# romz-pl/linear-programming-Vanderbei

Hardware: AMD Instinct MI355X
Metric: IPM iterations/sec (ADA^T factor+solve) on netlib dfl001; duality gap ≤1e-8 (higher is better)
Workload: dtype f64; 1 GPU; dfl001 hsd (BASELINE configs[2]), one step = one complete solve to mu < 1e-12; method=hsd, m=12155, n=12230, nz=71277, parallelism=replicas1, status=optimal solution, lnz=7160813, nsup=18147, levels=20, refine_passes=251

## Files before the change

### include/ipo_hip.h

```cpp
#ifndef IPO_HIP_H
#define IPO_HIP_H

#include <stdio.h>

#ifdef __cplusplus
extern "C" {
#endif

int solver(int m, int n, int nz, int *iA, int *kA, double *A, double *b, double *c, double f,
           double *x, double *y, double *w, double *z);

void ldltfac(int m, int n, int *kA, int *iA, double *A, double *dn, double *dm,
             int *kAt, int *iAt, double *At, int verbose);
void forwardbackward(double *Dn, double *Dm, double *dx, double *dy);
void inv_clo(void);
int ipo_hip_ldlt_set_q(int n, const int *kQ, const int *iQ, const double *Q, int max);

typedef struct {
    int    iters;
    int    status;
    double t_setup_s;
    double t_solve_s;
    double factor_ms;
    double solve_ms;
// ... 29 lines not shown
int  ipo_hip_ctx_run(ipo_hip_ctx *ctx, int method, int max_iter, FILE *trace, int timing, ipo_hip_stats *stats);
void ipo_hip_ctx_download(ipo_hip_ctx *ctx, double *x, double *y, double *w, double *z);
void ipo_hip_ctx_destroy(ipo_hip_ctx *ctx);
double ipo_hip_ctx_setup_seconds(const ipo_hip_ctx *ctx);

int ipo_hip_solve_qp(int m, int n, int nz, const int *iA, const int *kA, const double *A, const double *b,
                     const double *c, double f, const int *kQ, const int *iQ, const double *Q, double *x,
                     double *y, double *w, double *z, FILE *trace, int max_iter, int timing,
                     ipo_hip_stats *stats);
ipo_hip_ctx *ipo_hip_ctx_create_qp(int m, int n, const int *kA, const int *iA, const double *A,
                                   const double *b, const double *c, double f, const int *kQ, const int *iQ,
                                   const double *Q);

typedef int (*ipo_hip_allreduce_fn)(void *user, double *buf, long n, int op);
int ipo_hip_set_device(int device);
int ipo_hip_rccl_unique_id(void *out128);
ipo_hip_ctx *ipo_hip_ctx_create_shard(int m, int n, const int *kA, const int *iA, const double *A,
                                      const double *b, const double *c, double f, int nlink,
                                      int m_global, int n_global, long nz_global, int nranks, int rank,
                                      const void *rccl_id, ipo_hip_allreduce_fn fn, void *user);

int ipo_hip_run_mps(const char *path, int method, FILE *out, int timing, ipo_hip_stats *stats);

#define IPO_HIP_SPLIT_FREE 1
int ipo_hip_run_mps_ex(const char *path, int method, int flags, const char *solfile, FILE *out, int timing,
                       ipo_hip_stats *stats);

int ipo_hip_mps_dims(const char *path, int *m0, int *n0, int *nz0, int *m, int *n, int *nz);

int ipo_hip_mps_load(const char *path, int *m, int *n, int *nz, int *kA, int *iA, double *A,
                     double *b, double *c, double *f);

int ipo_hip_write_sol(const char *path, int flags, const double *x, const double *y, const double *z,
                      const char *solfile);

int ipo_hip_mps_quads(const char *path, int *n, int *qnz, int *kQ, int *iQ, double *Q);

int ipo_hip_mps_load_qp(const char *path, int *m, int *n, int *nz, int *kA, int *iA, double *A, double *b,
                        double *c, double *f, int *qnz, int *kQ, int *iQ, double *Q);

int ipo_hip_mps_load_ex(const char *path, int flags, int *m, int *n, int *nz, int *kA, int *iA, double *A,
                        double *b, double *c, double *f);

typedef struct ipo_hip_kkt ipo_hip_kkt;
ipo_hip_kkt *ipo_hip_kkt_create(int m, int n, const int *kA, const int *iA, const double *A);
ipo_hip_kkt *ipo_hip_kkt_create_q(int m, int n, const int *kA, const int *iA, const double *A, const int *kQ,
                                  const int *iQ, const double *Q, int qmax);
void   ipo_hip_kkt_destroy(ipo_hip_kkt *k);
int    ipo_hip_kkt_factor(ipo_hip_kkt *k, const double *E, const double *D);
int    ipo_hip_kkt_solve(ipo_hip_kkt *k, const double *E, const double *D, double *fy, double *fx);
int    ipo_hip_kkt_info(const ipo_hip_kkt *k, long *lnz, double *narth, int *nsup, int *nlevels, int *denwin,
                        int *pdf, double *epsdiag, int *ndep, int *passes);
int    ipo_hip_kkt_perm(const ipo_hip_kkt *k, int *perm);
int    ipo_hip_kkt_pivots(const ipo_hip_kkt *k, double *d, int *live);
void   ipo_hip_kkt_set_epsdiag(ipo_hip_kkt *k, double epsdiag);

int ipo_hip_symbolic(int m, int n, const int *kA, const int *iA, int *perm, long *lnz, double *narth,
                     int *denwin, int *pdf, int *nsup, int *nlevels);
int ipo_hip_symbolic_q(int m, int n, const int *kA, const int *iA, const int *kQ, const int *iQ, int *perm,
                       long *lnz, double *narth, int *denwin, int *pdf, int *nsup, int *nlevels);
int ipo_hip_symbolic_forced(int m, int n, const int *kA, const int *iA, int nforced, int *perm, int *colcount,
                            long *lnz, int *tail_c0, int *nsup, int *nlevels);
int ipo_hip_symbolic_tail(int m, int n, const int *kA, const int *iA, double density, int *tail_c0, int *nt,
                          int *ntb);

int ipo_hip_vector_bench(int m, int n, const int *kA, const int *iA, const double *A, int reps, double *ms3,
                         double *bytes3);

int ipo_hip_dot_ordered(const double *a, const double *b, int n, double *out);

int ipo_hip_q_times(int n, const int *kQ, const int *iQ, const double *Q, const double *v, int long_min,
                    double *out);
int ipo_hip_kkt_q_long(const ipo_hip_kkt *k);
int ipo_hip_ctx_q_long(const ipo_hip_ctx *ctx);

int ipo_hip_synth_random(int m, int n, int per_col, int band, unsigned long long seed, int *nz, int *kA, int *iA,
                         double *A, double *b, double *c, double *xs, double *ys, double *ws, double *zs);
int ipo_hip_synth_block_angular(int nblocks, int mb, int nb, int per_col, int band, int nlink, int link_nz,
                                unsigned long long seed, int *m, int *n, int *nz, int *kA, int *iA, double *A,
                                double *b, double *c, double *xs, double *ys, double *ws, double *zs);

int ipo_hip_tail_run_schedule(int nt, int K, int L, int cap, unsigned *items, int max_items, int *ptr);

long ipo_hip_kkt_schedule(int m, int n, const int *kA, const int *iA, int nforced, int cus, const char *name, int *out,
                          long cap);

int ipo_hip_device_count(void);
int ipo_hip_device_synchronize(void);
const char *ipo_hip_last_error(void);
const char *ipo_hip_version(void);

#ifdef __cplusplus
}
#endif
#endif
```

### linear-programming-vanderbei_amd/csrc/capi.cpp

```cpp
#include "../../include/ipo_hip.h"

#include <hip/hip_runtime.h>

#include <algorithm>
#include <cmath>
#include <cstdlib>
#include <cstring>
#include <memory>
#include <stdexcept>
#include <string>
#include <utility>
#include <vector>

#include "ipm.h"
#include "kkt_device.h"
#include "kkt_schedule.h"
#include "lp_io.h"
#include "synth.h"

namespace {

thread_local std::string g_err;

void set_err(const std::string& s) { g_err = s; }
// ... 733 lines not shown

int ipo_hip_device_synchronize(void) {
    const hipError_t e = hipDeviceSynchronize();
    if (e != hipSuccess) {
        set_err(std::string("hipDeviceSynchronize: ") + hipGetErrorString(e));
        return -1;
    }
    return 0;
}

const char* ipo_hip_last_error(void) { return g_err.c_str(); }
const char* ipo_hip_version(void) { return "ipo-hip 0.1 (gfx950)"; }

}

namespace {
std::vector<int> schedule_array(const ipo::KktPlan& P, const ipo::KktKnobs& knobs, const ipo::KktSchedule& S,
                                const std::string& name) {
    using V = std::vector<int>;
    const auto flat2 = [](const std::vector<ipo::SchedInt2>& w) {
        V v;
        for (const ipo::SchedInt2& e : w) { v.push_back(e.x); v.push_back(e.y); }
        return v;
    };
    const auto chars = [](const std::vector<char>& w) { return V(w.begin(), w.end()); };
    const auto one = [](size_t x) { return static_cast<int>(x); };
    const std::pair<const char*, const V*> direct[] = {
        {"plan.col0", &P.col0}, {"plan.rowptr", &P.rowptr}, {"plan.parent", &P.parent}, {"plan.level", &P.level},
        {"plan.level_ptr", &P.level_ptr}, {"plan.level_sups", &P.level_sups}, {"plan.sup_of", &P.sup_of},
        {"plan.yrow_ptr", &P.yrow_ptr}, {"plan.yrow_idx", &P.yrow_idx}, {"plan.unit_level_ptr", &P.unit_level_ptr},
        {"plan.unit_sup", &P.unit_sup}, {"plan.kslot", &P.kslot}, {"plan.kslot_ptr", &P.kslot_ptr},
        {"plan.tail_kslot_ptr", &P.tail_kslot_ptr},
        {"panels.fu_sup", &S.panels.fu_sup}, {"panels.fu_j", &S.panels.fu_j}, {"panels.small_sups", &S.panels.small_sups},
        {"panels.fu_ptr", &S.panels.fu_ptr}, {"panels.small_ptr", &S.panels.small_ptr},
        {"panels.small1_cnt", &S.panels.small1_cnt},
        {"chunks.chunk_sup", &S.chunks.chunk_sup}, {"chunks.chunk_r0", &S.chunks.chunk_r0},
        {"chunks.sup_chunk0", &S.chunks.sup_chunk0}, {"chunks.chunk_ptr", &S.chunks.chunk_ptr},
        {"order.sweep_sups", &S.order.sweep_sups}, {"order.leaf_cnt", &S.order.leaf_cnt},
        {"order.leaf8_cnt", &S.order.leaf8_cnt},
        {"sf.ybase", &S.sf.ybase}, {"sf.yrow_idx", &S.sf.yrow_idx}, {"sf.zbase", &S.sf.zbase}, {"sf.zpi", &S.sf.zpi},
        {"sf.need", &S.sf.need}, {"sf.par", &S.sf.par}, {"sf.ylate_ptr", &S.sf.ylate_ptr},
        {"sf.ylate_idx", &S.sf.ylate_idx}, {"sf.pre_col", &S.sf.pre_col}, {"sf.pre_ptr", &S.sf.pre_ptr},
        {"sf.pre_idx", &S.sf.pre_idx},
        {"visits.kslot", &S.visits.kslot}, {"visits.kptr", &S.visits.kptr}, {"visits.late_b", &S.visits.late_b},
        {"gather.ck_u", &S.gather.ck_u}, {"gather.ck_b", &S.gather.ck_b}, {"gather.ck_e", &S.gather.ck_e},
        {"gather.ck_part", &S.gather.ck_part}, {"gather.ck_q", &S.gather.ck_q}, {"gather.sp_u", &S.gather.sp_u},
        {"gather.sp_p0", &S.gather.sp_p0}, {"gather.sp_n", &S.gather.sp_n}, {"gather.ck_ptr", &S.gather.ck_ptr},
        {"gather.sp_ptr", &S.gather.sp_ptr}, {"gather.ck_kind", &S.gather.ck_kind},
        {"tail.visit_ptr", &S.tail.visit_ptr}, {"tail.run_ptr", &S.tail.run_ptr},
    };
    for (const auto& d : direct)
        if (name == d.first) return *d.second;
    if (name == "plan.dims") return {P.T, P.nsup, P.nlevels, P.tail_c0, P.nt, P.ntb};
    if (name == "plan.task_src") {
        V v;
        for (const ipo::TailTask& t : P.utasks) v.push_back(t.src);
        return v;
    }
    if (name == "paths")
        return {S.paths.visits, S.paths.chain_lead, S.paths.tail_run, S.paths.run_winpub, S.paths.small_leaves,
                S.paths.sf_width};
    if (name == "panels.split_level") return chars(S.panels.split_level);
    if (name == "sf.items_f") return flat2(S.sf.items_f);
    if (name == "sf.items_b") return flat2(S.sf.items_b);
    if (name == "sf.dims") return {S.sf.sf_level, one(S.sf.ybuf_stride), one(S.sf.zpad_stride), S.sf.late_lists};
    if (name == "visits.vis") {
        V v;
        for (size_t g = 0; g < S.visits.vis.size(); g++)
            for (const ipo::SchedInt3& e : S.visits.vis[g]) v.insert(v.end(), {one(g), e.x, e.y, e.z});
        return v;
    }
    if (name == "gather.ck_wide") return chars(S.gather.ck_wide);
    if (name == "gather.dims") return {one(S.gather.split_cnt), one(S.gather.partial_tiles)};
    if (name == "chunks.dims") return {one(S.chunks.partial_stride)};
    if (name == "work.launches") return {S.work.fwd_launches, S.work.bwd_launches};
    const auto steps = [](const std::vector<ipo::SweepStep>& w) {
        V v;
        for (const ipo::SweepStep& e : w) v.insert(v.end(), {e.kind, e.q0, e.n, e.a, e.b});
        return v;
    };
    if (name == "sweep.fwd") return steps(S.sweep.fwd);
    if (name == "sweep.bwd") return steps(S.sweep.bwd);
    if (name == "sweep.split") return {S.sweep.split};
    if (name == "sweep.fwd_blocked" || name == "sweep.bwd_blocked") {
        const ipo::SweepSteps b = ipo::build_sweep_steps(P, knobs, S.paths, S.chunks, S.order, S.sf, true);
        return steps(name == "sweep.fwd_blocked" ? b.fwd : b.bwd);
    }
    if (name == "tail.visit_list") return V(S.tail.visit_list.begin(), S.tail.visit_list.end());
    if (name == "tail.run_items") {
        V v;
        for (const ipo::SchedUint2& e : S.tail.run_items) { v.push_back(static_cast<int>(e.x)); v.push_back(static_cast<int>(e.y)); }
        return v;
    }
    throw std::invalid_argument("kkt_schedule: unknown array '" + name + "'");
}

void synth_out(const ipo::SynthLP& o, int* kA, int* iA, double* A, double* b, double* c, double* xs, double* ys,
               double* ws, double* zs) {
    std::copy(o.kA.begin(), o.kA.end(), kA);
    std::copy(o.iA.begin(), o.iA.end(), iA);
    std::copy(o.A.begin(), o.A.end(), A);
    std::copy(o.b.begin(), o.b.end(), b);
    std::copy(o.c.begin(), o.c.end(), c);
    if (xs) std::copy(o.xs.begin(), o.xs.end(), xs);
    if (ys) std::copy(o.ys.begin(), o.ys.end(), ys);
    if (ws) std::copy(o.ws.begin(), o.ws.end(), ws);
    if (zs) std::copy(o.zs.begin(), o.zs.end(), zs);
}
}

extern "C" {

int ipo_hip_vector_bench(int m, int n, const int* kA, const int* iA, const double* A, int reps, double* ms3,
                         double* bytes3) {
    try {
        ipo::vector_bench(m, n, kA, iA, A, reps, ms3, bytes3);
        return 0;
    } catch (const std::exception& e) {
        set_err(e.what());
        return -1;
    }
}

int ipo_hip_tail_run_schedule(int nt, int K, int L, int cap, unsigned* items, int max_items, int* ptr) {
    try {
        if (nt <= 0 || K <= 0 || L <= 0 || cap <= 1) throw std::invalid_argument("tail_schedule: bad arguments");
        const int ntb = (nt + ipo::kPanelCols - 1) / ipo::kPanelCols;
        if (ntb > ipo::kTailSchedMaxBlocks)
            throw std::invalid_argument("tail_schedule: nt gives " + std::to_string(ntb) + " block columns, the limit is " +
                                        std::to_string(ipo::kTailSchedMaxBlocks));
        std::vector<int> pv;
        const std::vector<ipo::SchedUint2> v = ipo::tail_run_schedule(ntb, nt, K, L, cap, pv);
        const int n = static_cast<int>(v.size());
        if (items)
            for (int i = 0; i < std::min(n, max_items); i++) {
                items[2 * i] = v[i].x;
                items[2 * i + 1] = v[i].y;
            }
        if (ptr) std::copy(pv.begin(), pv.end(), ptr);
        return n;
    } catch (const std::exception& e) {
        set_err(e.what());
        return -1;
    }
}

long ipo_hip_kkt_schedule(int m, int n, const int* kA, const int* iA, int nforced, int cus, const char* name, int* out,
                          long cap) {
    try {
        if (!name || cus <= 0) throw std::invalid_argument("kkt_schedule: bad arguments");
        std::vector<int> kat, iat;
        std::vector<double> at, a(kA[n], 1.0);
        ipo::csc_transpose(m, n, kA, iA, a.data(), kat, iat, at);
        const ipo::KktPlan P =
            ipo::build_kkt_plan(m, n, kA, iA, kat.data(), iat.data(), nforced, ipo::device_tail_density());
        const ipo::KktKnobs knobs = ipo::KktKnobs::from_env();
        const ipo::KktSchedule S = ipo::build_kkt_schedule(P, knobs, cus);
        const std::string names(name);
        std::vector<int> v;
        if (names.find(',') == std::string::npos) {
            v = schedule_array(P, knobs, S, names);
        } else {
            for (size_t b = 0; b <= names.size();) {
                const size_t e = std::min(names.find(',', b), names.size());
                const std::vector<int> w = schedule_array(P, knobs, S, names.substr(b, e - b));
                v.push_back(static_cast<int>(w.size()));
                v.insert(v.end(), w.begin(), w.end());
                b = e + 1;
            }
        }
        if (out) std::copy(v.begin(), v.begin() + std::min<long>(cap, static_cast<long>(v.size())), out);
        return static_cast<long>(v.size());
    } catch (const std::exception& e) {
        set_err(e.what());
        return -1;
    }
}

int ipo_hip_dot_ordered(const double* a, const double* b, int n, double* out) {
    try {
        if (n < 0 || (n > 0 && (!a || !b)) || !out) throw std::invalid_argument("dot_ordered: bad arguments");
        *out = ipo::dot_ordered_host(a, b, n);
        return 0;
    } catch (const std::exception& e) {
        set_err(e.what());
        return -1;
    }
}

int ipo_hip_q_times(int n, const int* kQ, const int* iQ, const double* Q, const double* v, int long_min,
                    double* out) {
    try {
        if (n < 0 || !kQ || !out || (n > 0 && !v)) throw std::invalid_argument("q_times: bad arguments");
        if (kQ[0] != 0) throw std::invalid_argument("q_times: kQ[0] != 0");
        for (int j = 0; j < n; j++)
            if (kQ[j + 1] < kQ[j]) throw std::invalid_argument("q_times: kQ decreasing at column " + std::to_string(j));
        if (n > 0 && kQ[n] > 0 && (!iQ || !Q)) throw std::invalid_argument("q_times: bad arguments");
        for (int k = 0; k < (n > 0 ? kQ[n] : 0); k++)
            if (iQ[k] < 0 || iQ[k] >= n) throw std::invalid_argument("q_times: row index out of range at entry " + std::to_string(k));
        const int thr = long_min > 0 ? long_min : ipo::KktKnobs::from_env().q_long;
        ipo::q_times_host(n, kQ, iQ, Q, v, thr, out);
        return 0;
    } catch (const std::exception& e) {
        set_err(e.what());
        return -1;
    }
}

int ipo_hip_kkt_q_long(const ipo_hip_kkt* k) { return k->kkt->q_long_count(); }

int ipo_hip_ctx_q_long(const ipo_hip_ctx* ctx) { return ctx->solver->kkt().q_long_count(); }

int ipo_hip_synth_random(int m, int n, int per_col, int band, unsigned long long seed, int* nz, int* kA, int* iA,
                         double* A, double* b, double* c, double* xs, double* ys, double* ws, double* zs) {
    try {
        if (nz) *nz = static_cast<int>(static_cast<long long>(n) * per_col);
        if (!kA) return 0;
        ipo::SynthLP o;
        ipo::synth_random(m, n, per_col, band, seed, o);
        synth_out(o, kA, iA, A, b, c, xs, ys, ws, zs);
        return 0;
    } catch (const std::exception& e) {
        set_err(e.what());
// ... 25 lines not shown
```

### linear-programming-vanderbei_amd/csrc/kkt_dense.hip

```cpp
#include <hip/hip_runtime.h>

#include <algorithm>
#include <cmath>
#include <stdexcept>

#include "dev_common.h"
#include "hip_util.h"
#include "kkt_kernels.h"

namespace ipo {

namespace {

struct DiagCtx {
    double* dscale;
    double* dg;
    int* live;
    int* flags;
    const int* sign;
    double tau;
};

__device__ __forceinline__ bool factor_diag_fast(const DiagCtx p, double* panel, int ld, int nc, int c0,
                                                 double (*B)[PC + 1]) {
// ... 877 lines not shown
            __builtin_amdgcn_s_setprio(3);
            if (cw0 + WIN <= nc) win_solve<true, DEP>(a, cw0, nc, rok, lane, Ct, Lb, dv, S.prog + w, prog + w, ds);
            else win_solve<false, DEP>(a, cw0, nc, rok, lane, Ct, Lb, dv, S.prog + w, prog + w, ds);
            if (SC && rp.pub && kb + 1 < tv.ntb) {
                bool ok = true;
                if (!DEP) {
                    for (int v = 0; v <= w; v++) {
                        int x;
                        while ((x = __hip_atomic_load(S.wverd + v, __ATOMIC_RELAXED, __HIP_MEMORY_SCOPE_WORKGROUP)) == 0)
                            __builtin_amdgcn_s_sleep(1);
                        ok = ok && x == 1;
                    }
                }
                if (ok && kb - 1 > rp.t0) {
                    const int need = max(1, (tv.nt - (kb - 1) * PC + TR - 1) / TR - 1);
                    int got = 0;
                    if (lane == 0) {
                        for (;;) {
                            got = sc1_load_int(rp.pread + kb - 1);
                            if (got >= need) break;
                            const int b = sc1_load_int(p.flags + 2);
                            if (b && b - 1 < kb) break;
                            __builtin_amdgcn_s_sleep(1);
                        }
                    }
                    ok = __builtin_amdgcn_readfirstlane(got) >= need;
                }
                if (ok) {
                    double* pb = rp.pub + (((size_t)(kb & 1) * tv.ntb + j) * 4 + w) * kTailPubWin;
                    if (rok) {
#pragma unroll
                        for (int q = 0; q < WIN; q++)
                            if (cw0 + q < nc) sc1_store(pb + q * TR + lane, a[q]);
                    }
                    if (lane < WIN) sc1_store(pb + WIN * TR + lane, dv[cw0 + lane]);
                    asm volatile("s_waitcnt vmcnt(0)" ::: "memory");
                    if (lane == 0)
                        __hip_atomic_store(rp.wflag_w + ((size_t)kb * tv.ntb + j) * 4 + w, rp.epoch, __ATOMIC_RELAXED,
                                           __HIP_MEMORY_SCOPE_AGENT);
                }
            }
        }
        __builtin_amdgcn_s_setprio(0);
        PANEL_STAMP(2);
        if (wbuf && (h1 ? rok : (j == 0 && lane >= nc && lane < h0))) {
            double dw[WIN];
            win_row(&dv[cw0], dw);
#pragma unroll
            for (int q = 0; q < WIN; q++) {
                const int c = cw0 + q;
                if (c < nc) wbuf[row + (size_t)c * ld] = a[q] * dw[q];
            }
        }
    }
    __builtin_amdgcn_fence(__ATOMIC_RELEASE, "workgroup", "local");
    __builtin_amdgcn_s_barrier();
    __builtin_amdgcn_fence(__ATOMIC_ACQUIRE, "workgroup", "local");
    if (winpub && !pre_wait()) return false;
    PANEL_STAMP(12);
    if (!DEP && tiny_sh && dep) return true;
    const bool fail = DEP ? (S.spec > 0 || (S.spec < 0 && S.ndep > 0 && [&] {
                                 for (int k = 0; k < nc; k++)
                                     if (!S.lv[k]) return true;
                                 return false;
                             }()))
                          : tiny_sh != 0;
    if (fail) {
        if (tid == 0) {
            atomicOr(&p.flags[1], fu_sup ? 2 : DEP ? 4 | 16 : 4);
            if (!fu_sup) atomicMax(&p.flags[2], kb + 1);
            if (DEP && !fu_sup && j == 0)
                __hip_atomic_store(p.flags + 3, 0, __ATOMIC_RELAXED, __HIP_MEMORY_SCOPE_AGENT);
        }
        post(true);
        return false;
    }
    if (w < nwin && (h1 ? rok && tile : (j == 0 && lane >= nc && lane < h0))) {
#pragma unroll
        for (int q = 0; q < WIN; q++) {
            const int c = cw0 + q;
            if (c < nc) st_h<SC>(panel + row + (size_t)c * ld, a[q]);
        }
    }
    if (j == 0 && tid < nc) { st_h<SC>(p.dg + c0 + tid, dv[tid]); p.live[c0 + tid] = DEP ? S.lv[tid] != 0 : 1; }
    post(false);
    if (!fu_sup && pre && j == 0 && !h1 && lane < nc && (lane >> 4) == w) st_h<SC>(p.dscale + c0 + lane, dsc_pre);
    if (j != 0) return false;
    if (!h1) {
#pragma unroll
        for (int q = 0; q < WIN; q++) Ct[lane][cw0 + q] = a[q];
    }
    __syncthreads();
    for (int rr = 1 + wv; rr < nc; rr += PNT / 64)
        if (lane < rr) st_h<SC>(panel + lane + (size_t)rr * ld, Ct[rr][lane]);
    if (DEP && tid == 0) {
        if (S.ndep) atomicAdd(&p.flags[0], S.ndep);
        if (!fu_sup)
            __hip_atomic_store(p.flags + 3, S.ndep, __ATOMIC_RELAXED, __HIP_MEMORY_SCOPE_AGENT);
    }
    PANEL_STAMP(13);
    return false;
}

__global__ void __launch_bounds__(PNT)
k_panel_w(PlanView p, const int* __restrict__ fu_sup, const int* __restrict__ fu_j, int f0, TailView tv, int kb) {
    __shared__ __attribute__((aligned(16))) char lds[sizeof(PanelLds)];
    PanelLds& S = *reinterpret_cast<PanelLds*>(lds);
    const int dep = fu_sup ? (tv.sdep ? 1 : 0) : 0;
    if (panel_w_body<false>(p, fu_sup, fu_j, f0, tv, kb, blockIdx.x, S, tv.W, false, nullptr, 0, dep)) {
        __syncthreads();
        panel_w_body<true>(p, fu_sup, fu_j, f0, tv, kb, blockIdx.x, S, tv.W, false, nullptr, 0, dep);
    }
}


constexpr int SKS = PC + 16;
struct SyrkLds {
    double As[PC][SKS];
    double Bs[PC][SKS];
};

template <int S>
__device__ __forceinline__ double diag_terms(const double (*As)[S], const double (*Bs)[S], int r, int nc, double as) {
    int k = 0;
    for (; k + 16 <= nc; k += 16) {
        double pr[16];
#pragma unroll
        for (int u = 0; u < 16; u++) pr[u] = fabs(As[k + u][r] * Bs[k + u][r]);
#pragma unroll
        for (int u = 0; u < 16; u++) as += pr[u];
    }
    for (; k < nc; k++) as += fabs(As[k][r] * Bs[k][r]);
    return as;
}
__device__ __forceinline__ double diag_terms(const SyrkLds& L, int r, int nc, double as) {
    return diag_terms<SKS>(L.As, L.Bs, r, nc, as);
}

__device__ __forceinline__ void mfma_32x16(const SyrkLds& L, int wr, int wc, int li, int lk, double4_t (&acc)[2]) {
#pragma unroll
    for (int kk = 0; kk < PC; kk += 4) {
        double av[2];
#pragma unroll
        for (int a = 0; a < 2; a++) av[a] = L.As[kk + lk][wr + a * 16 + li];
        const double bv = L.Bs[kk + lk][wc + li];
#pragma unroll
        for (int a = 0; a < 2; a++) acc[a] = __builtin_amdgcn_mfma_f64_16x16x4f64(av[a], bv, acc[a], 0, 0, 0);
    }
}

#ifdef IPO_VISIT_STAMPS
__device__ long long g_vstamps[8][16][6];
#define VISIT_STAMP(blk, slot)                                                                          \
    do {                                                                                                \
        if (blockIdx.x == 0 && (threadIdx.x & 63) == 0 && (blk) < 16)                                   \
            g_vstamps[threadIdx.x >> 6][(blk)][(slot)] = clock64();                                     \
    } while (0)
#else
#define VISIT_STAMP(blk, slot) do {} while (0)
#endif

__device__ __forceinline__ void syrk_tile512(const PlanView& p, const TailView& tv, int kb, int bi, int bj,
                                             SyrkLds& L) {
    const int nt = tv.nt, k0 = kb * PC, nc = min(PC, nt - k0), tid = threadIdx.x;
    const double* Lcol = tv.S + (size_t)k0 * nt;
    {
        double va[TR * PC / PNT], vb[TR * PC / PNT];
// ... 119 lines not shown
        __syncthreads();
        VISIT_STAMP(b - b0, 2);
        if (b + 1 < b1) load(b + 1, xx, yy, dd);
        VISIT_STAMP(b - b0, 3);
        mfma_32x16(L, wr, wc, li, lk, acc);
        VISIT_STAMP(b - b0, 4);
        if (diag_tile && tid < TR) as = diag_terms(L, tid, min(PC, nt - b * PC), as);
        __syncthreads();
        VISIT_STAMP(b - b0, 5);
    };
    for (int b = b0; b < b1; b++) step(b, rx, ry, rd);
#pragma unroll
    for (int a = 0; a < 2; a++)
#pragma unroll
        for (int i = 0; i < 4; i++) L.As[wc + (lane & 15)][wr + a * 16 + (lane >> 4) + 4 * i] = acc[a][i];
    __syncthreads();
#pragma unroll
    for (int u = 0; u < 8; u++) {
        const int cc = wv + 8 * u, cg = bj * TR + cc;
        if (rgl < nt && cg < nt && !(diag_tile && cc > lane)) st_h<SC>(tv.S + rgl + (size_t)cg * nt, old[u] - L.As[cc][lane]);
    }
    if (diag_tile && tid < TR && bi * TR + tid < nt) {
        double* dp = p.dscale + tv.tc + bi * TR + tid;
        st_h<SC>(dp, ld_h<SC>(dp) + as);
    }
}

constexpr size_t kTailStepLds0 = sizeof(PanelLds) > sizeof(SyrkLds) ? sizeof(PanelLds) : sizeof(SyrkLds);
constexpr size_t kTailStepLds = kTailStepLds0 > sizeof(PreLds) ? kTailStepLds0 : sizeof(PreLds);

__global__ void __launch_bounds__(PNT)
k_tail_pr(PlanView p, TailView tv, int t, int gp, int vbase) {
    __shared__ __attribute__((aligned(16))) char lds[kTailStepLds];
    if ((int)blockIdx.x < gp) {
        PanelLds& S = *reinterpret_cast<PanelLds*>(lds);
        if (panel_w_body<false>(p, nullptr, nullptr, 0, tv, t, blockIdx.x, S, nullptr, t > 0, p.flags + 2, t, tv.dep)) {
            __syncthreads();
            panel_w_body<true>(p, nullptr, nullptr, 0, tv, t, blockIdx.x, S, nullptr, t > 0, p.flags + 2, t, tv.dep);
        }
        return;
    }
    if (tv.vlist) {
        const unsigned v = tv.vlist[vbase + blockIdx.x - gp];
        visit_tile512(p, tv, v & 255, (v >> 8) & 255, (v >> 16) & 255, v >> 24, *reinterpret_cast<SyrkLds*>(lds),
                      p.flags + 2, t);
        return;
    }
    int tile = blockIdx.x - gp, c = t + 1;
    while (tile >= tv.ntb - c) { tile -= tv.ntb - c; c++; }
    const int b1 = visit_hi(t, c, tv.vk);
    visit_tile512(p, tv, c + tile, c, max(0, b1 - tv.vk), b1, *reinterpret_cast<SyrkLds*>(lds), p.flags + 2, t);
}

__host__ __device__ __forceinline__ int tail_gp(int nt, int t) { return max(1, (nt - t * PC + TR - 1) / TR - 1); }

__global__ void __launch_bounds__(PNT)
k_tail_run(PlanView p, TailView tv, TailRun rc) {
    __shared__ __attribute__((aligned(16))) char lds[kTailStepLds];
    __shared__ int sh_item, sh_ok, sh_ok2;
    const int ntb = tv.ntb;
    const int* bailp = p.flags + 2;
    if (threadIdx.x == 0) sh_item = __hip_atomic_fetch_add(rc.ticket, 1, __ATOMIC_RELAXED, __HIP_MEMORY_SCOPE_AGENT);
    __syncthreads();
    const int it = sh_item;
    if (it >= rc.n) return;
    const uint2 rec = rc.items[it];
    const int t = rec.y & 0xff, q = (rec.y >> 8) & 0xff;
    unsigned long long* tr = rc.trace ? rc.trace + 4 * (size_t)it : nullptr;
    if (tr && threadIdx.x == 0) {
        tr[0] = __builtin_amdgcn_s_memrealtime();
        tr[3] = __builtin_amdgcn_s_getreg((20 << 0) | (0 << 6) | (3 << 11));
    }
    if (rec.y >> 31) {
        const int j = rec.x;
        const int* vd = q ? rc.vseq + t * ntb + t : nullptr;
        const int* vt = q && t + j + 1 < ntb ? rc.vseq + (t + j + 1) * ntb + t : nullptr;
        const bool winpub = rc.pub && t > 0 && t - 1 >= rc.t0;
        if (!winpub && !run_wait(vd, q, vt, q, bailp, t, &sh_ok)) return;
        auto pw = [&]() {
            const bool go = t == rc.t0 || run_wait(rc.pdone + t - 1, tail_gp(tv.nt, t - 1), nullptr, 0, bailp, t, &sh_ok2);
            if (tr && threadIdx.x == 0) tr[1] = __builtin_amdgcn_s_memrealtime();
            return go;
        };
        auto post = [&](bool bailed) { run_signal(rc.pdone + t, bailed ? 1 + kRunBail : 1); };
        if (tr && threadIdx.x == 0 && t == 0) tr[1] = __builtin_amdgcn_s_memrealtime();
        PanelLds& S = *reinterpret_cast<PanelLds*>(lds);
        const RunPub rp{rc.pub, rc.wflag, rc.wflag, rc.pread, rc.t0, rc.epoch, vd, vt, q, &sh_ok};
        if (panel_w_body<false, true>(p, nullptr, nullptr, 0, tv, t, j, S, nullptr, t > 0, nullptr, t, tv.dep, pw,
                                      post, rp)) {
            __syncthreads();
            panel_w_body<true, true>(p, nullptr, nullptr, 0, tv, t, j, S, nullptr, t > 0, nullptr, t, tv.dep, NoWait{},
                                     post, rp);
        }
    } else {
        const int bi = rec.x & 255, c = (rec.x >> 8) & 255, b0 = (rec.x >> 16) & 255, b1 = rec.x >> 24;
        int* vs = rc.vseq + bi * ntb + c;
        if (!run_wait(t > rc.t0 ? rc.pdone + t - 1 : nullptr, t > rc.t0 ? tail_gp(tv.nt, t - 1) : 0, q ? vs : nullptr,
                      q, bailp, t, &sh_ok))
            return;
        if (tr && threadIdx.x == 0) tr[1] = __builtin_amdgcn_s_memrealtime();
        visit_tile512<true>(p, tv, bi, c, b0, b1, *reinterpret_cast<SyrkLds*>(lds));
        run_signal(vs);
    }
    if (tr && threadIdx.x == 0) tr[2] = __builtin_amdgcn_s_memrealtime();
}

__global__ void __launch_bounds__(256)
k_tail_restore(PlanView p, TailView tv, int kb) {
    const int nt = tv.nt, k0 = kb * PC, nc = min(PC, nt - k0), h = nt - k0, c = blockIdx.y;
    double* panel = tv.S + k0 + (size_t)k0 * nt;
    for (int row = nc + blockIdx.x * 256 + threadIdx.x; row < h; row += gridDim.x * 256)
        panel[row + (size_t)c * nt] = tv.W[row + (size_t)c * nt];
    if (blockIdx.x == 0 && c == 0) {
        if ((int)threadIdx.x < nc) p.dscale[tv.tc + k0 + threadIdx.x] = tv.W[threadIdx.x];
        if (threadIdx.x == 0) {
            p.flags[0] -= p.flags[3];
            p.flags[3] = 0;
        }
    }
}

__global__ void __launch_bounds__(PNT)
k_tail_col(PlanView p, TailView tv, int t) {
    __shared__ __attribute__((aligned(16))) char lds[sizeof(SyrkLds)];
    syrk_tile512(p, tv, t, t + 1 + blockIdx.x, t + 1, *reinterpret_cast<SyrkLds*>(lds));
}

constexpr int SNC = 16;

__device__ __forceinline__ void panel_s_body(const PlanView& p, const int* __restrict__ sups, int q0, int q, int dep) {
    const int lane = threadIdx.x & 63;
    const int s = sups[q0 + q];
    const int c0 = p.col0[s], nc = p.col0[s + 1] - c0;
    const int h = nc + (p.rowptr[s + 1] - p.rowptr[s]), ld = h;
    double* panel = p.Lx + p.off[s];
    const bool rok = lane < h;
    double a[SNC];
#pragma unroll
    for (int c = 0; c < SNC; c++) {
        const bool ok = rok && c < nc && c <= lane;
        const double t = panel[ok ? lane + (size_t)c * ld : 0];
        a[c] = ok ? t : 0.0;
    }
    double dsc = lane < nc ? p.dscale[c0 + lane] : 0.0;
    double mydv = 0.0;
    int mylive = 1, ndep = 0;
#pragma unroll
    for (int k = 0; k < SNC; k++) {
        if (k < nc) {
            double dk = lane_bcast(a[k], k);
            const double dsk = lane_bcast(dsc, k);
            int alive = 1;
            if (fabs(dk) <= p.tau * dsk) {
                const bool in = lane > k && rok;
                const bool nan = __ballot(in && a[k] != a[k]) != 0;
                if (!dep || nan) {
                    if (lane == 0) atomicOr(&p.flags[1], 8);
                    return;
                }
                if (__ballot(in && !(fabs(a[k]) < 1.0e+6 * 1.0e-8)) != 0) dk = (p.sign[c0 + k] < 0 ? -1.0 : 1.0) * 1.0e-8;
                else alive = 0;
                ndep++;
            }
            mylive = lane == k ? alive : mylive;
            const bool below = lane > k && rok;
            const double l = alive && below ? a[k] / dk : 0.0;
            a[k] = below ? l : a[k];
            mydv = lane == k ? dk : mydv;
            const double c = l * dk;
            dsc = dsc + fabs(l * c);
#pragma unroll
            for (int qq = k + 1; qq < SNC; qq++)
                if (qq < nc) a[qq] = a[qq] - l * lane_bcast(c, qq);
        }
    }
    if (rok) {
// ... 154 lines not shown
```

### linear-programming-vanderbei_amd/csrc/kkt_device.h

```cpp
#pragma once
#include <hip/hip_runtime.h>

#include <cstddef>
#include <cstdint>
#include <memory>
#include <vector>

#include "hip_util.h"
#include "exchange.h"
#include "kkt_knobs.h"
#include "kkt_plan.h"
#include "kkt_schedule.h"

namespace ipo {

struct TailView {
    double* S;
    int nt, ntb, tc;
    const int* task_ptr;
    const TailTask* tasks;
    double* W;
    int vk = kTailVisitBlocks;
    int dep = 1;
    const unsigned* vlist = nullptr;
    const int* vptr = nullptr;
    int sdep = 1;
};

struct TailRun {
    const uint2* items;
    int n;
    int t0;
    int* ticket;
    int* pdone;
    int* vseq;
    double* pub = nullptr;
    int* wflag = nullptr;
    int* pread = nullptr;
    int epoch = 0;
    unsigned long long* trace = nullptr;
};

constexpr int kTailPubWin = 16 * 64 + 16;

struct KktTimers {
    double phase_ms[kNumPhases] = {};
    long phase_launches[kNumPhases] = {};
    long phase_count[kNumPhases] = {};
    double factor_ms = 0.0;
    double solve_ms = 0.0;
    double sweep_ms = 0.0;
    long factors = 0, solves = 0, rawsolves = 0;
    long panel_redos = 0;
    long redo_where[4] = {0, 0, 0, 0};
    long tail_repairs = 0;
    long tail_dep_rounds = 0;
};

struct QBlock {
    const int* kQ = nullptr;
    const int* iQ = nullptr;
    const double* Q = nullptr;
    int qmax = 1;
};

struct PlanView;

class KktDevice {
  public:
    KktDevice(int m, int n, const int* kA, const int* iA, const double* A, hipStream_t stream, int nforced = 0,
              const QBlock* qb = nullptr);
    ~KktDevice();
    KktDevice(const KktDevice&) = delete;
    KktDevice& operator=(const KktDevice&) = delete;

    const KktPlan& plan() const { return plan_; }
    void set_exchange(Exchange* x) { xch_ = x; }
    int nforced() const { return nforced_; }
    int m() const { return m_; }
    int n() const { return n_; }
    hipStream_t stream() const { return stream_; }

    const int* kA() const { return dkA_.get(); }
    const int* iA() const { return diA_.get(); }
    const double* A() const { return dA_.get(); }
    const int* kAt() const { return dkAt_.get(); }
    const int* iAt() const { return diAt_.get(); }
    const double* At() const { return dAt_.get(); }
    const int* kQ() const { return qnz_ > 0 ? dkQ_.get() : nullptr; }
    const int* iQ() const { return qnz_ > 0 ? diQ_.get() : nullptr; }
    const double* Q() const { return qnz_ > 0 ? dQ_.get() : nullptr; }
    int q_long_count() const { return q_long_n_; }
    int q_long_min() const { return q_long_n_ > 0 ? knobs_.q_long : 0; }
    void launch_q_long(const double* v, double* out);

    struct PrePass {
        int R = 0;
        double* dfy[2] = {nullptr, nullptr};
        double* dfx[2] = {nullptr, nullptr};
        hipStream_t stream = nullptr;
        hipEvent_t ready = nullptr;
    };
    void factor(const double* dE, const double* dD, const PrePass* pre = nullptr);
    int solve(const double* dE, const double* dD, double* dfy, double* dfx);
    int solve2(const double* dE, const double* dD, double* dfy1, double* dfx1, double* dfy2, double* dfx2);
    void solve_multi(int R, const double* dE, const double* dD, double* const* dfy, double* const* dfx, int* ok);

    void rawsolve(double* dz, int R = 1, size_t fwd_first = 0);

    struct HostState {
        double epsdiag;
        int ndep;
        KktTimers tm;
    };
    HostState host_state() const { return {epsdiag_, ndep_, tm_}; }
    void restore_host_state(const HostState& h) { epsdiag_ = h.epsdiag; ndep_ = h.ndep; tm_ = h.tm; drop_prepass(); }

    double epsdiag() const { return epsdiag_; }
// ... 30 lines not shown
    PlanView plan_view() const;
    bool tail_repair() const { return use_panel_ && !xch_ && knobs_.tail_repair; }
    void factor_core(const double* dE, const double* dD, const PrePass* pre);
    void dump_factor(const double* dE, const double* dD, double eps_in);
    int dump_count_ = 0;
    TailView tail_view() const;
    template <int R>
    void sweep(double* dz, const double* epsp, size_t fwd_first);
    template <int R>
    int run_sweep_steps(const std::vector<SweepStep>& steps, bool forward, double* dz, const double* epsp,
                        size_t first = 0, size_t last = SIZE_MAX, hipStream_t s = nullptr);
    void tail_rhs_begin(double* dz, int R);
    void tail_rhs_end(double* dz, int R);
    DevBuf<int> dIncons_;
    int launch_gather(const struct PlanView& pv, const TailView& tv, int tail, int group, hipStream_t s);
    void launch_reduce_maxabs2(const double* a, int na, const double* b, int nb, double* dst);

    int m_, n_, T_;
    int nforced_ = 0;
    Exchange* xch_ = nullptr;
    DevBuf<double> dLinkAx_;
    int long_row0_ = -1;
    DevBuf<double> dLongAx_;
    bool shard_minor() const { return xch_ && xch_->rank() != 0; }
    void xsum(double* d, size_t n, RedOp op) { if (xch_) xch_->allreduce(d, n, op, stream_); }
    hipStream_t stream_;
    KktPlan plan_;
    double epsdiag_ = 1.0e-14;
    int ndep_ = 0;
    double pivot_tol_ = knobs_.pivtol;
    int last_passes_ = 0;
    bool timing_ = false;
    KktTimers tm_;
    hipEvent_t ev0_ = nullptr, ev1_ = nullptr, ev2_ = nullptr, ev3_ = nullptr;
    std::vector<hipEvent_t> kev_;
    size_t kev_used_ = 0;
    struct PhaseMark { hipEvent_t b, e; int phase, launches; };
    std::vector<PhaseMark> marks_;
    hipEvent_t mark_b_ = nullptr;
    hipEvent_t next_event();
    void ph_begin(hipStream_t s);
    void ph_end(int phase, int launches, hipStream_t s);
    void ph_collect();
  public:
    double work_flops[kNumPhases] = {}, work_bytes[kNumPhases] = {};
  private:

    DevBuf<int> dkA_, diA_, dkAt_, diAt_;
    DevBuf<double> dA_, dAt_;
    int qnz_ = 0, qmax_ = 1;
    DevBuf<int> dkQ_, diQ_;
    DevBuf<double> dQ_, dQdiag_;
    DevBuf<int64_t> dqmap_;
    int q_long_n_ = 0;
    DevBuf<int> dQLongCols_;
    DevBuf<double> dLongQ_;
    DevBuf<int> dcol0_, drowptr_, drows_, dperm_, diperm_;
    DevBuf<int64_t> doff_, damap_, ddslot_, drelptr_;
    DevBuf<int> dunit_sup_, dunit_tile_, dtask_ptr_, dtask_pair_, dtask_i0_, dtask_i1_;
    DevBuf<int> dupd_src_, dupd_r0_, dupd_r1_, drel_, dlevel_sups_;
    DevBuf<int> dyrow_ptr_, dyrow_idx_;
    DevBuf<int> dylate_ptr_, dylate_idx_, dpre_col_, dpre_ptr_, dpre_idx_;
    DevBuf<double> dYbuf_;
    int sf_grid_ = 1;
    int sf_fwd_epoch_ = 0, sf_bwd_epoch_ = 0;
    long long sf_ticket_next_[2] = {0, 0};
#ifdef IPO_SF_STAMPS
    std::vector<SchedInt2> h_sf_items_f_;
#endif
    int sf_tbase(int d, int nitems, hipStream_t s);
    DevBuf<int2> dsf_items_f_, dsf_items_b_;
    DevBuf<int> dsf_need_, dsf_par_, dsf_zbase_, dsf_zpi_, dsf_fcnt_, dsf_fflag_, dsf_bcnt_, dsf_bflag_, dsf_ticket_;
    DevBuf<int> dybase_;
    DevBuf<double> dZpad_;
    DevBuf<int> dfu_sup_, dfu_j_;
    DevBuf<int> dsmall_sups_;
    const bool use_panel_ = knobs_.panel;
    bool factor_pass(const double* dE, const double* dD, bool fused, bool tail_fused, const PrePass* pre = nullptr);
    bool prepass_eligible(const PrePass* pre, bool fused, bool tail_fused) const;
    void enqueue_prepass(const PrePass& pre);
    void run_prepass_steps(int R, hipStream_t q);
    void enqueue_pass_head(int R, double* const* dfy, double* const* dfx, double* part, hipStream_t s);
    bool take_prepass(int R, double* const* dfy, double* const* dfx);
    void drop_prepass() { if (pre_state_ != kPreNone) { pre_state_ = kPreNone; pre_discarded_++; } }
    enum { kPreNone = 0, kPreEnqueued, kPreValid };
    int pre_state_ = kPreNone;
    PrePass pre_req_;
    hipEvent_t ev_pre_fork_ = nullptr, ev_pre_done_ = nullptr;
    long pre_used_ = 0, pre_discarded_ = 0;
    DevBuf<double> dPrePart_;
    void enqueue_levels(const PlanView& pv, const TailView& tv, bool fused, hipStream_t s, const PrePass* pre);
    bool finish_pass(bool fused);
    void repair_tail();
    DevBuf<int> dsweep_sups_;
    DevBuf<int> dchunk_sup_, dchunk_r0_, dsup_chunk0_;
    DevBuf<double> dPartial_;
    int gst_group_ = knobs_.gather_stamps, gst_n_ = 0;
    DevBuf<long long> dGStamp_;
    DevBuf<int> dck_u_, dck_b_, dck_e_, dck_part_, dsp_u_, dsp_p0_, dsp_n_;
    DevBuf<int> dck_q_;
    DevBuf<int> dSplitCnt_;
    bool eps_cleared_ = false;
    DevBuf<double> dPartialTile_;
    DevBuf<TaskSrc> dusrc_, dtsrc_;
    DevBuf<SlotRec> dslot_rec_, dtail_slot_rec_;
    DevBuf<unsigned long long> dChainGran_;
    int chain_epoch_ = 0;
    DevBuf<int> dtail_task_ptr_, dtail_kslot_, dtail_kslot_ptr_;
    DevBuf<int> dlead_ticket_;
    long long lead_ticket_next_ = 0;
    DevBuf<unsigned> dvisit_list_;
    DevBuf<uint2> drun_items_;
    DevBuf<int> drun_cnt_;
    DevBuf<double> drun_pub_;
    DevBuf<int> drun_wflag_;
    int run_epoch_ = 0;
    void launch_tail_from(int t0, bool reset);
    DevBuf<uint64_t> dtail_tasks_, dutasks_;
    DevBuf<double> dW_;
    DevBuf<double> dDepSt_;
    DevBuf<int> dDepI_;
    DevBuf<double> dLx_, dDg_;
    DevBuf<int> dLive_;
    DevBuf<double> dDscale_;
    DevBuf<int> dFlags_;
    DevBuf<double> dZ_, dDy_, dDx_, dRy_, dRx_;
    DevBuf<double> dPart_, dScal_;
    DevBuf<double> dFacScal_;
    double* hScal_ = nullptr;
    int* hFlags_ = nullptr;
};

}
```

### linear-programming-vanderbei_amd/csrc/kkt_device.hip

```cpp
#include <hip/hip_runtime.h>

#include <chrono>
#include <algorithm>
#include <cmath>
#include <cstdio>
#include <cstdlib>
#include <cstring>

#include "dev_common.h"
#include "kkt_device.h"
#include "kkt_kernels.h"
#include "lp_io.h"

namespace ipo {

namespace {

__global__ void __launch_bounds__(NT)
k_assemble_A(int nz, const double* __restrict__ A, const int64_t* __restrict__ amap, double* __restrict__ Lx) {
    const int k = blockIdx.x * NT + threadIdx.x;
    if (k < nz) Lx[amap[k]] = A[k];
}

__global__ void __launch_bounds__(NT)
// ... 841 lines not shown
SweepOrder KktDevice::build_sweep_order(const SolveChunks& ch) {
    hipStream_t s = stream_;
    SweepOrder so = ipo::build_sweep_order(plan_, h_.paths, ch);
    dsweep_sups_.upload(so.sweep_sups, s);
    IPO_HIP_CHECK(hipStreamSynchronize(s));
    so.sweep_sups = {};
    return so;
}

void KktDevice::build_gather_chunks(const VisitSlots& vs) {
    hipStream_t s = stream_;
    GatherChunks g = ipo::build_gather_chunks(plan_, knobs_, h_.paths, vs);
    dck_u_.upload(g.ck_u, s);
    dck_b_.upload(g.ck_b, s);
    dck_e_.upload(g.ck_e, s);
    dck_part_.upload(g.ck_part, s);
    dsp_u_.upload(g.sp_u, s);
    dsp_p0_.upload(g.sp_p0, s);
    dsp_n_.upload(g.sp_n, s);
    dck_q_.upload(g.ck_q, s);
    dSplitCnt_.alloc(g.split_cnt);
    IPO_HIP_CHECK(hipMemsetAsync(dSplitCnt_.get(), 0, g.split_cnt * sizeof(int), s));
    dPartialTile_.alloc(g.partial_tiles * (kTileRows * kTileRows + 4 * kTileRows));
    IPO_HIP_CHECK(hipStreamSynchronize(s));
    h_.ck_ptr = std::move(g.ck_ptr);
    h_.ck_kind = std::move(g.ck_kind);
    h_.ck_wide = std::move(g.ck_wide);
}

void KktDevice::count_work() {
    const WorkCounts w = ipo::count_work(plan_, knobs_, h_.sweep);
    std::copy(w.flops, w.flops + kNumPhases, work_flops);
    std::copy(w.bytes, w.bytes + kNumPhases, work_bytes);
}

void KktDevice::build_slot_records(const std::vector<int>& kslot_v) {
    hipStream_t s = stream_;
    auto build = [&](const std::vector<TailTask>& ts, DevBuf<TaskSrc>& dst) {
        const std::vector<TaskSrc> v = build_task_src(plan_, ts);
        dst.upload(v, s);
        IPO_HIP_CHECK(hipStreamSynchronize(s));
    };
    build(plan_.utasks, dusrc_);
    if (plan_.nt > 0) build(plan_.tail_tasks, dtsrc_);
    auto expand = [&](const std::vector<int>& kslot, const std::vector<TailTask>& ts, DevBuf<SlotRec>& dst) {
        const std::vector<SlotRec> v = ipo::build_slot_records(plan_, kslot, ts);
        dst.upload(v, s);
        IPO_HIP_CHECK(hipStreamSynchronize(s));
    };
    expand(h_.paths.visits ? kslot_v : plan_.kslot, plan_.utasks, dslot_rec_);
    if (plan_.nt > 0) expand(plan_.tail_kslot, plan_.tail_tasks, dtail_slot_rec_);
    dutasks_.upload(reinterpret_cast<const uint64_t*>(plan_.utasks.data()), plan_.utasks.size() * 4, s);
}

void KktDevice::setup_tail(int cus) {
    hipStream_t s = stream_;
    if (plan_.nt > 0) {
        dtail_task_ptr_.upload(plan_.tail_task_ptr, s);
        dtail_kslot_.upload(plan_.tail_kslot, s);
        dtail_kslot_ptr_.upload(plan_.tail_kslot_ptr, s);
        static_assert(sizeof(TailTask) == 32, "TailTask layout");
        dtail_tasks_.upload(reinterpret_cast<const uint64_t*>(plan_.tail_tasks.data()), plan_.tail_tasks.size() * 4, s);
        dW_.alloc(static_cast<size_t>(plan_.nt) * kPanelCols);
        dDepSt_.alloc(tail_dep_state_doubles(plan_.ntb));
        dDepI_.alloc(8);
        dChainGran_.alloc(static_cast<size_t>(plan_.ntb) * (2 * 128 + 2 * 4 * 64 * 2));
        dlead_ticket_.alloc(1);
        IPO_HIP_CHECK(hipMemsetAsync(dlead_ticket_.get(), 0, sizeof(int), s));
        lead_ticket_next_ = 0;
        IPO_HIP_CHECK(hipMemsetAsync(dChainGran_.get(), 0, dChainGran_.bytes(), s));
    }
    raise_sweep_lds(false);
    if (plan_.nt > 0 && plan_.ntb <= kTailSchedMaxBlocks) {
        TailSchedule ts = build_tail_schedule(plan_, knobs_, h_.paths, cus);
        if (knobs_.visit_sched) {
            dvisit_list_.upload(ts.visit_list, s);
            IPO_HIP_CHECK(hipStreamSynchronize(s));
            h_.visit_ptr = std::move(ts.visit_ptr);
        }
        if (h_.paths.tail_run) {
            static_assert(sizeof(SchedUint2) == sizeof(uint2), "SchedUint2 is uploaded as uint2");
            drun_items_.upload(reinterpret_cast<const uint2*>(ts.run_items.data()), ts.run_items.size(), s);
            h_.run_ptr = std::move(ts.run_ptr);
            drun_cnt_.alloc(1 + plan_.ntb + static_cast<size_t>(plan_.ntb) * plan_.ntb + plan_.ntb);
            if (h_.paths.run_winpub) {
                drun_pub_.alloc(2 * static_cast<size_t>(plan_.ntb) * 4 * kTailPubWin);
                drun_wflag_.alloc(static_cast<size_t>(plan_.ntb) * plan_.ntb * 4);
                IPO_HIP_CHECK(hipMemsetAsync(drun_wflag_.get(), 0, drun_wflag_.bytes(), s));
                run_epoch_ = 0;
            }
            IPO_HIP_CHECK(hipStreamSynchronize(s));
        }
    }
}

void KktDevice::alloc_numeric() {
    hipStream_t s = stream_;
    dLx_.alloc(plan_.lx_size > 0 ? plan_.lx_size : 1);
    dDg_.alloc(T_ > 0 ? T_ : 1);
    dLive_.alloc(T_ > 0 ? T_ : 1);
    dDscale_.alloc(T_ > 0 ? T_ : 1);
    dFlags_.alloc(4 + T_);
    {
        std::vector<int> fl(4 + T_, 0);
        for (int v = 0; v < T_; v++) fl[4 + v] = plan_.dsign[v];
        dFlags_.upload(fl, s);
    }
    dZ_.alloc(2 * (T_ > 0 ? T_ : 1));
    dDy_.alloc(2 * (m_ > 0 ? m_ : 1));
    dRy_.alloc(2 * (m_ > 0 ? m_ : 1));
    dDx_.alloc(2 * (n_ > 0 ? n_ : 1));
    dRx_.alloc(2 * (n_ > 0 ? n_ : 1));
    dIncons_.alloc(2);
    dPart_.alloc(8 * kRedBlocks);
    dScal_.alloc(16);
    dFacScal_.alloc(8);
    dPrePart_.alloc(8 * kRedBlocks);
    IPO_HIP_CHECK(hipHostMalloc(reinterpret_cast<void**>(&hScal_), 16 * sizeof(double), hipHostMallocDefault));
    IPO_HIP_CHECK(hipHostMalloc(reinterpret_cast<void**>(&hFlags_), 8 * sizeof(int), hipHostMallocDefault));
    IPO_HIP_CHECK(hipEventCreate(&ev0_));
    IPO_HIP_CHECK(hipEventCreate(&ev1_));
    IPO_HIP_CHECK(hipEventCreate(&ev2_));
    IPO_HIP_CHECK(hipEventCreate(&ev3_));
    IPO_HIP_CHECK(hipEventCreateWithFlags(&ev_pre_fork_, hipEventDisableTiming));
    IPO_HIP_CHECK(hipEventCreateWithFlags(&ev_pre_done_, hipEventDisableTiming));
    IPO_HIP_CHECK(hipStreamSynchronize(s));
}

void KktDevice::build_sync_free_plan(const SolveChunks& ch, const SweepOrder& so, int cus) {
    hipStream_t s = stream_;
    dyrow_ptr_.upload(plan_.yrow_ptr, s);
    const SyncFreePlan sf = ipo::build_sync_free_plan(plan_, knobs_, h_.paths, ch);
    const int ns = plan_.nsup;
    h_.sf_level = sf.sf_level;
    dyrow_idx_.upload(sf.yrow_idx, s);
    dybase_.upload(sf.ybase, s);
    if (sf.late_lists) {
        dylate_ptr_.upload(sf.ylate_ptr, s);
        dylate_idx_.upload(sf.ylate_idx.empty() ? std::vector<int>{0} : sf.ylate_idx, s);
        dpre_col_.upload(sf.pre_col.empty() ? std::vector<int>{0} : sf.pre_col, s);
        dpre_ptr_.upload(sf.pre_ptr, s);
        dpre_idx_.upload(sf.pre_idx.empty() ? std::vector<int>{0} : sf.pre_idx, s);
        IPO_HIP_CHECK(hipStreamSynchronize(s));
    }
    h_.ybuf_stride = sf.ybuf_stride;
    dYbuf_.alloc(2 * h_.ybuf_stride);
    h_.sweep = build_sweep_steps(plan_, knobs_, h_.paths, ch, so, sf, h_.paths.tail_blocked);
    if (sf.range(plan_)) {
        static_assert(sizeof(SchedInt2) == sizeof(int2), "SchedInt2 is uploaded as int2");
        dsf_items_f_.upload(reinterpret_cast<const int2*>(sf.items_f.data()), sf.items_f.size(), s);
#ifdef IPO_SF_STAMPS
        h_sf_items_f_ = sf.items_f;
#endif
        dsf_items_b_.upload(reinterpret_cast<const int2*>(sf.items_b.data()), sf.items_b.size(), s);
        dsf_need_.upload(sf.need, s);
        dsf_par_.upload(sf.par, s);
        dsf_zbase_.upload(sf.zbase, s);
        dsf_zpi_.upload(sf.zpi, s);
        h_.zpad_stride = sf.zpad_stride;
        dZpad_.alloc(2 * h_.zpad_stride);
        for (DevBuf<int>* b : {&dsf_fcnt_, &dsf_fflag_, &dsf_bcnt_, &dsf_bflag_}) {
            b->alloc(ns);
            IPO_HIP_CHECK(hipMemsetAsync(b->get(), 0, ns * sizeof(int), s));
        }
        dsf_ticket_.alloc(2);
        IPO_HIP_CHECK(hipMemsetAsync(dsf_ticket_.get(), 0, 2 * sizeof(int), s));
        sf_ticket_next_[0] = sf_ticket_next_[1] = 0;
        sf_grid_ = cus;
    }
    raise_sweep_lds(true);
    IPO_HIP_CHECK(hipStreamSynchronize(s));
}

KktDevice::~KktDevice() {
    dump_sf_stamps();
    if (knobs_.debug_redo)
        std::fprintf(stderr, "kkt: %ld factorisations, %ld redone; bails (unused) %ld, k_panel_w sparse %ld, tail %ld, "
                             "k_panel_s %ld; tail block columns repaired %ld in %ld rounds\n", tm_.factors,
                     tm_.panel_redos, tm_.redo_where[0], tm_.redo_where[1], tm_.redo_where[2], tm_.redo_where[3],
                     tm_.tail_repairs, tm_.tail_dep_rounds);
    if (knobs_.debug_redo)
        std::fprintf(stderr, "kkt: forward pre-passes used %ld, discarded %ld\n", pre_used_, pre_discarded_);
    if (hScal_) (void)hipHostFree(hScal_);
    if (hFlags_) (void)hipHostFree(hFlags_);
    if (ev0_) (void)hipEventDestroy(ev0_);
    if (ev1_) (void)hipEventDestroy(ev1_);
    if (ev2_) (void)hipEventDestroy(ev2_);
    if (ev3_) (void)hipEventDestroy(ev3_);
    if (ev_pre_fork_) (void)hipEventDestroy(ev_pre_fork_);
    if (ev_pre_done_) (void)hipEventDestroy(ev_pre_done_);
    for (hipEvent_t e : kev_) (void)hipEventDestroy(e);
}

PlanView KktDevice::plan_view() const {
    PlanView v;
    v.col0 = dcol0_.get(); v.rowptr = drowptr_.get(); v.rows = drows_.get(); v.off = doff_.get();
    v.unit_sup = dunit_sup_.get(); v.unit_tile = dunit_tile_.get();
    v.task_ptr = dtask_ptr_.get(); v.task_pair = dtask_pair_.get();
    v.task_i0 = dtask_i0_.get(); v.task_i1 = dtask_i1_.get();
    v.upd_src = dupd_src_.get(); v.upd_r0 = dupd_r0_.get(); v.upd_r1 = dupd_r1_.get();
    v.relptr = drelptr_.get(); v.rel = drel_.get();
    v.Lx = dLx_.get(); v.dg = dDg_.get(); v.live = dLive_.get();
    v.flags = dFlags_.get();
    v.sign = dFlags_.get() + 4;
    v.xcd = knobs_.update_xcd;
    v.dscale = dDscale_.get();
    v.tau = pivot_tol_;
    v.incons = dIncons_.get();
    v.ybase = dybase_.get();
    return v;
}

TailView KktDevice::tail_view() const {
    TailView t;
    t.S = dLx_.get() + plan_.off_tail;
    t.nt = plan_.nt;
    t.ntb = plan_.ntb;
    t.tc = plan_.tail_c0;
    t.task_ptr = dtail_task_ptr_.get();
    t.tasks = reinterpret_cast<const TailTask*>(dtail_tasks_.get());
    t.W = dW_.get();
    t.vk = knobs_.visit_blocks;
    if (!h_.visit_ptr.empty()) {
        t.vlist = dvisit_list_.get();
        t.vptr = h_.visit_ptr.data();
    }
    t.dep = tail_repair() ? knobs_.tail_spec : 0;
    t.sdep = knobs_.sparse_dep;
    return t;
}

void KktDevice::dump_factor(const double* dE, const double* dD, double eps_in) {
    if (knobs_.dump_dir.empty()) return;
    std::vector<double> E(m_), D(n_), dg(T_), dsc(T_);
    std::vector<int> live(T_);
    IPO_HIP_CHECK(hipStreamSynchronize(stream_));
    if (m_) IPO_HIP_CHECK(hipMemcpy(E.data(), dE, m_ * sizeof(double), hipMemcpyDeviceToHost));
    if (n_) IPO_HIP_CHECK(hipMemcpy(D.data(), dD, n_ * sizeof(double), hipMemcpyDeviceToHost));
    dLive_.download(live.data(), T_, stream_);
    dDg_.download(dg.data(), T_, stream_);
    dDscale_.download(dsc.data(), T_, stream_);
    IPO_HIP_CHECK(hipStreamSynchronize(stream_));
    char path[4096];
    std::snprintf(path, sizeof path, "%s/f%04d.bin", knobs_.dump_dir.c_str(), dump_count_++);
    FILE* f = std::fopen(path, "wb");
    if (!f) return;
    const int hdr[4] = {m_, n_, T_, ndep_};
    const double eps[2] = {eps_in, epsdiag_};
    std::fwrite(hdr, sizeof(int), 4, f);
    std::fwrite(eps, sizeof(double), 2, f);
    std::fwrite(E.data(), sizeof(double), m_, f);
    std::fwrite(D.data(), sizeof(double), n_, f);
    std::fwrite(plan_.perm.data(), sizeof(int), T_, f);
    std::fwrite(live.data(), sizeof(int), T_, f);
    std::fwrite(dg.data(), sizeof(double), T_, f);
    std::fwrite(dsc.data(), sizeof(double), T_, f);
    std::fclose(f);
}

void KktDevice::factor(const double* dE, const double* dD, const PrePass* pre) {
    const double eps_in = epsdiag_;
    drop_prepass();
    try {
        factor_core(dE, dD, pre);
    } catch (...) {
        if (pre_state_ != kPreNone) (void)hipStreamWaitEvent(stream_, ev_pre_done_, 0);
        drop_prepass();
        throw;
    }
    dump_factor(dE, dD, eps_in);
}

void KktDevice::factor_core(const double* dE, const double* dD, const PrePass* pre) {
// ... 28 lines not shown
        if (plan_.off_tail > 0) IPO_HIP_CHECK(hipMemsetAsync(dLx_.get(), 0, plan_.off_tail * sizeof(double), s));
        hipLaunchKernelGGL(k_zero_tail_lower, dim3(plan_.nt), dim3(NT), 0, s, dLx_.get() + plan_.off_tail, plan_.nt);
    } else {
        IPO_HIP_CHECK(hipMemsetAsync(dLx_.get(), 0, dLx_.bytes(), s));
    }
    if (nz > 0) hipLaunchKernelGGL(k_assemble_A, dim3(ceil_div(nz, NT)), dim3(NT), 0, s, nz, dA_.get(), damap_.get(), dLx_.get());
    if (qnz_ > 0)
        hipLaunchKernelGGL(k_assemble_Q, dim3(ceil_div(qnz_, NT)), dim3(NT), 0, s, qnz_, dQ_.get(), dqmap_.get(),
                           static_cast<double>(qmax_), dLx_.get());
    hipLaunchKernelGGL(k_assemble_diag, dim3(ceil_div(T_, NT)), dim3(NT), 0, s, T_, m_, dperm_.get(), dE, dD, epsdiag_,
                       ddslot_.get(), dLx_.get(), dLive_.get(), dDscale_.get(), shard_minor() ? plan_.tail_c0 : T_,
                       dFlags_.get(), dkQ_.get() ? dQdiag_.get() : static_cast<const double*>(nullptr),
                       static_cast<double>(qmax_));
    const TailView tv = tail_view();
    if (!prepass_eligible(pre, fused, tail_fused)) pre = nullptr;
    enqueue_levels(pv, tv, fused, s, pre);
    if (plan_.nt > 0) {
        xsum(tv.S, static_cast<size_t>(plan_.nt) * plan_.nt, RedOp::Sum);
        xsum(dDscale_.get() + plan_.tail_c0, plan_.nt, RedOp::Sum);
        if (tail_fused && h_.paths.tail_run) {
            launch_tail_from(0, true);
        } else if (tail_fused) {
            ph_begin(s);
            for (int t = 0; t < plan_.ntb; t++) launch_tail_step(pv, tv, t, s);
            ph_end(kPhTail, plan_.ntb, s);
        } else
        for (int kb = 0; kb < plan_.ntb; kb++) {
            const int k0 = kb * kPanelCols, nc = std::min(kPanelCols, plan_.nt - k0);
            const int below = plan_.nt - k0 - nc;
            ph_begin(s);
            {
                launch_diag(pv, nullptr, 0, 1, tv, kb, s);
                ph_end(kPhDiag, 1, s);
                if (below > 0) {
                    ph_begin(s);
                    launch_trsm(pv, 0, -1, tv, kb, s);
                    ph_end(kPhTrsm, 1, s);
                }
            }
            if (below > 0) {
                const int nb = plan_.ntb - kb - 1;
                ph_begin(s);
                hipLaunchKernelGGL(k_tail_syrk, dim3(nb * (nb + 1) / 2), dim3(NT), 0, s, pv, tv, kb);
                ph_end(kPhSyrk, 1, s);
            }
        }
    }
    if (pre) IPO_HIP_CHECK(hipStreamWaitEvent(s, ev_pre_done_, 0));
    return finish_pass(fused || tail_fused);
}

bool KktDevice::prepass_eligible(const PrePass* pre, bool fused, bool tail_fused) const {
    return knobs_.prepass && pre && (pre->R == 1 || pre->R == 2) && pre->stream && pre->stream != stream_ &&
           pre->ready && fused && tail_fused && h_.paths.tail_run && h_.sweep.split > 0 && !xch_ && !timing_;
}

void KktDevice::enqueue_pass_head(int R, double* const* dfy, double* const* dfx, double* part, hipStream_t s) {
    RedJobs j{};
    j.nj = 2 * R;
    PermJobs J{};
    for (int r = 0; r < R; r++) {
        j.a[2 * r] = dfx[r]; j.b[2 * r] = nullptr; j.len[2 * r] = n_; j.op[2 * r] = 1;
        j.a[2 * r + 1] = dfy[r]; j.b[2 * r + 1] = nullptr; j.len[2 * r + 1] = m_; j.op[2 * r + 1] = 1;
        J.fy[r] = dfy[r];
        J.fx[r] = dfx[r];
        J.z[r] = dZ_.get() + static_cast<size_t>(r) * T_;
    }
    launch_reduce(j, part, dScal_.get() + 8, s);
    xsum(dScal_.get() + 8, 2 * R, RedOp::Max);
    hipLaunchKernelGGL(k_perm_in2, dim3(ceil_div(T_, NT), R), dim3(NT), 0, s, T_, m_, dperm_.get(), J, dIncons_.get(),
                       dScal_.get() + 4);
}

void KktDevice::enqueue_prepass(const PrePass& pre) {
    hipStream_t q = pre.stream;
    IPO_HIP_CHECK(hipEventRecord(ev_pre_fork_, stream_));
    IPO_HIP_CHECK(hipStreamWaitEvent(q, ev_pre_fork_, 0));
    IPO_HIP_CHECK(hipStreamWaitEvent(q, pre.ready, 0));
    enqueue_pass_head(pre.R, pre.dfy, pre.dfx, dPrePart_.get(), q);
    run_prepass_steps(pre.R, q);
    IPO_HIP_CHECK(hipEventRecord(ev_pre_done_, q));
    pre_req_ = pre;
    pre_state_ = kPreEnqueued;
}

void KktDevice::enqueue_levels(const PlanView& pv, const TailView& tv, bool fused, hipStream_t s, const PrePass* pre) {
    for (int l = 0; l < plan_.nlevels; l++) {
        const int u0 = plan_.unit_level_ptr[l], u1 = plan_.unit_level_ptr[l + 1];
        if (u1 <= u0) continue;
        if (l > 0) {
            ph_begin(s);
            const int nl = launch_gather(pv, tv, -1, l, s);
            ph_end(kPhGather, nl, s);
        }
        const int q0 = plan_.level_ptr[l], q1 = plan_.level_ptr[l + 1];
        ph_begin(s);
        if (fused && h_.split_level[l]) {
            launch_diag(pv, dlevel_sups_.get(), q0, q1 - q0, tv, 0, s);
            launch_trsm(pv, u0, u1 - u0, tv, 0, s);
            ph_end(kPhDiag, 2, s);
        } else if (fused) {
            const int nsm = h_.small_ptr[l + 1] - h_.small_ptr[l], nfu = h_.fu_ptr[l + 1] - h_.fu_ptr[l];
            const int n1 = h_.small1_cnt[l];
            if (knobs_.merge_levels && nfu > 0 && nsm > n1) {
                launch_panel_small(pv, dsmall_sups_.get(), h_.small_ptr[l], n1, tv.sdep, s, n1);
                launch_panel_ws(pv, dfu_sup_.get(), dfu_j_.get(), h_.fu_ptr[l], nfu, tv, dsmall_sups_.get(),
                                h_.small_ptr[l] + n1, nsm - n1, tv.sdep, s);
                ph_end(kPhDiag, 1 + (n1 > 0), s);
            } else {
                launch_panel_small(pv, dsmall_sups_.get(), h_.small_ptr[l], nsm, tv.sdep, s, n1);
                launch_panel(pv, dfu_sup_.get(), dfu_j_.get(), h_.fu_ptr[l], nfu, tv, -1, s);
                ph_end(kPhDiag, (nsm > 0) + (nfu > 0), s);
            }
        } else {
            launch_diag(pv, dlevel_sups_.get(), q0, q1 - q0, tv, 0, s);
            ph_end(kPhDiag, 1, s);
            ph_begin(s);
            launch_trsm(pv, u0, u1 - u0, tv, 0, s);
            ph_end(kPhTrsm, 1, s);
        }
    }
    if (pre) enqueue_prepass(*pre);
    if (plan_.nt > 0) {
        ph_begin(s);
        const int nl = launch_gather(pv, tv, 0, plan_.nlevels, s);
        ph_end(kPhGather, nl, s);
    }
}

bool KktDevice::finish_pass(bool fused) {
    hipStream_t s = stream_;
    IPO_HIP_CHECK(hipGetLastError());
    hipLaunchKernelGGL(k_min_abs_partial, dim3(kRedBlocks), dim3(NT), 0, s, dDg_.get(), T_, dPart_.get());
    if (xch_) {
        hipLaunchKernelGGL(k_finish_reduce, dim3(1), dim3(kRedThreads), 0, s, dPart_.get(), 1, 1u, dFacScal_.get());
        hipLaunchKernelGGL(k_flag_to_scalar, dim3(1), dim3(1), 0, s, dFlags_.get(), dFacScal_.get() + 1);
        hipLaunchKernelGGL(k_flag_to_scalar, dim3(1), dim3(1), 0, s, dFlags_.get() + 1, dFacScal_.get() + 2);
        xsum(dFacScal_.get(), 3, RedOp::Max);
        hipLaunchKernelGGL(k_pack_ints, dim3(1), dim3(3), 0, s, dFlags_.get(), 3, dFacScal_.get() + 3);
    } else {
        hipLaunchKernelGGL(k_finish_reduce_pack, dim3(1), dim3(kRedThreads), 0, s, dPart_.get(), 1, 1u, dFacScal_.get(),
                           static_cast<const int*>(dFlags_.get()), 3, dFacScal_.get() + 3);
    }
    IPO_HIP_CHECK(hipMemcpyAsync(hScal_, dFacScal_.get(), 5 * sizeof(double), hipMemcpyDeviceToHost, s));
    if (timing_) IPO_HIP_CHECK(hipEventRecord(ev1_, s));
    IPO_HIP_CHECK(hipStreamSynchronize(s));
    if (gst_n_ > 0) {
        std::vector<long long> st(1024 * 8);
        IPO_HIP_CHECK(hipMemcpy(st.data(), dGStamp_.get(), st.size() * sizeof(long long), hipMemcpyDeviceToHost));
        long long t0 = st[0];
        for (int b = 0; b < std::min(gst_n_, 1024); b++) t0 = std::min(t0, st[b * 8]);
        std::fprintf(stderr, "gather stamps group %d, %d workgroups (us from first start: start rec val mfma acc put slots)\n",
                     gst_group_, gst_n_);
        for (int b = 0; b < std::min(gst_n_, 1024); b++) {
            const long long* q = st.data() + b * 8;
            std::fprintf(stderr, "  wg %4d: %6.2f %6.2f %6.2f %6.2f %6.2f %6.2f  %lld\n", b, (q[0] - t0) / 100.0,
                         (q[1] - t0) / 100.0, (q[2] - t0) / 100.0, (q[3] - t0) / 100.0, (q[4] - t0) / 100.0,
                         (q[5] - t0) / 100.0, q[6]);
        }
        gst_n_ = 0;
        gst_group_ = -1;
    }
    {
        int f[3];
        std::memcpy(f, hScal_ + 3, sizeof(f));
        hFlags_[0] = f[0];
        hFlags_[1] = f[1];
        hFlags_[4] = f[2];
    }
    if (timing_) {
        float ms = 0;
        IPO_HIP_CHECK(hipEventElapsedTime(&ms, ev0_, ev1_));
        tm_.factor_ms += ms;
        ph_collect();
    }
    const bool bail = xch_ ? hScal_[2] > 0 : hFlags_[1] != 0;
    return !(fused && bail);
}

void KktDevice::launch_tail_from(int t0, bool reset) {
    hipStream_t s = stream_;
    const PlanView pv = plan_view();
    const size_t ncnt = reset ? drun_cnt_.size() : 1;
    IPO_HIP_CHECK(hipMemsetAsync(drun_cnt_.get(), 0, ncnt * sizeof(int), s));
    TailRun rc;
    rc.items = drun_items_.get() + h_.run_ptr[t0];
    rc.n = h_.run_ptr[plan_.ntb] - h_.run_ptr[t0];
    rc.t0 = t0;
    rc.ticket = drun_cnt_.get();
    rc.pdone = drun_cnt_.get() + 1;
    rc.vseq = drun_cnt_.get() + 1 + plan_.ntb;
    if (h_.paths.run_winpub) {
        if (run_epoch_ == INT_MAX) {
            IPO_HIP_CHECK(hipMemsetAsync(drun_wflag_.get(), 0, drun_wflag_.bytes(), s));
            run_epoch_ = 0;
        }
        rc.pub = drun_pub_.get();
        rc.wflag = drun_wflag_.get();
        rc.pread = rc.vseq + static_cast<size_t>(plan_.ntb) * plan_.ntb;
        if (!reset) IPO_HIP_CHECK(hipMemsetAsync(rc.pread + t0, 0, (plan_.ntb - t0) * sizeof(int), s));
        rc.epoch = ++run_epoch_;
    }
    ph_begin(s);
    launch_tail_run(pv, tail_view(), rc, s);
    ph_end(kPhTail, rc.n > 0, s);
}

void KktDevice::repair_tail() {
    hipStream_t s = stream_;
    const PlanView pv = plan_view();
    for (;;) {
        const int tb = hFlags_[4] - 1;
        tm_.tail_repairs++;
        if (timing_) IPO_HIP_CHECK(hipEventRecord(ev0_, s));
        IPO_HIP_CHECK(hipMemsetAsync(dFlags_.get() + 1, 0, 2 * sizeof(int), s));
        TailView tv = tail_view();
        if (hFlags_[1] & 16) launch_tail_restore(pv, tv, tb, s);
        ph_begin(s);
        if (tb > 0) launch_tail_colupdate(pv, tv, tb - 1, s);
        ph_end(kPhTail, tb > 0, s);
        IPO_HIP_CHECK(hipMemsetAsync(dDepI_.get(), 0, 8 * sizeof(int), s));
        constexpr int kDepBatch = 4;
        for (int r = 0;; r += kDepBatch) {
            if (r > kPanelCols + 1) throw std::runtime_error("kkt: dense-tail dependent-pivot rounds did not finish");
            ph_begin(s);
            for (int b = 0; b < kDepBatch; b++)
                launch_tail_dep_round(pv, tv, tb, r + b, dDepSt_.get(), dDepI_.get(), s);
            ph_end(kPhTail, kDepBatch, s);
            IPO_HIP_CHECK(hipMemcpyAsync(hFlags_ + 6, dDepI_.get() + 4 * ((r + kDepBatch) & 1) + 2, sizeof(int),
                                         hipMemcpyDeviceToHost, s));
            IPO_HIP_CHECK(hipStreamSynchronize(s));
            tm_.tail_dep_rounds += kDepBatch;
            if (hFlags_[6]) break;
        }
        if (h_.paths.tail_run) {
            launch_tail_from(tb + 1, false);
        } else {
            ph_begin(s);
            for (int t = tb + 1; t < plan_.ntb; t++) launch_tail_step(pv, tail_view(), t, s);
            ph_end(kPhTail, plan_.ntb - tb - 1, s);
        }
        if (finish_pass(true)) break;
        if ((hFlags_[1] & ~16) != 4 || hFlags_[4] - 1 <= tb)
            throw std::runtime_error("kkt: dense-tail repair did not advance");
    }
}

int KktDevice::launch_gather(const PlanView& pv, const TailView& tv, int tail, int group, hipStream_t s) {
    const int c0 = h_.ck_ptr[group], c1 = h_.ck_ptr[group + 1];
    if (c1 <= c0) return 0;
    const SlotRec* recs = tail < 0 ? dslot_rec_.get() : dtail_slot_rec_.get();
    long long* stq = nullptr;
    if (gst_group_ == group && tail < 0 && h_.ck_kind[group] > 0) {
        if (!dGStamp_.get()) dGStamp_.alloc(1024 * 8);
        stq = dGStamp_.get();
        gst_n_ = c1 - c0;
    }
    if (h_.ck_kind[group] == 2) {
        hipLaunchKernelGGL(k_update_quad, dim3(c1 - c0), dim3(NT), 0, s, pv, tv, recs, dck_u_.get(), dck_b_.get(),
                           dck_e_.get(), dck_part_.get(), c0, stq);
        return 1;
    }
    if (h_.ck_kind[group] == 1) {
        if (h_.ck_wide[group])
        hipLaunchKernelGGL(k_update_flat<4>, dim3(c1 - c0), dim3(NT), 0, s, pv, tv, tail, recs, dck_u_.get(),
                           dck_b_.get(), dck_e_.get(), dck_part_.get(), c0, dPartialTile_.get(), dck_q_.get(),
                           dsp_p0_.get(), dsp_n_.get(), dSplitCnt_.get(), stq);
        else
        hipLaunchKernelGGL(k_update_flat<1>, dim3(c1 - c0), dim3(NT), 0, s, pv, tv, tail, recs, dck_u_.get(),
                           dck_b_.get(), dck_e_.get(), dck_part_.get(), c0, dPartialTile_.get(), dck_q_.get(),
                           dsp_p0_.get(), dsp_n_.get(), dSplitCnt_.get(), stq);
        return 1;
    }
    const int occ = knobs_.update_occ;
    auto go = [&](auto kern) {
        hipLaunchKernelGGL(kern, dim3(c1 - c0), dim3(NT), 0, s, pv, tv, tail, recs, dck_u_.get(), dck_b_.get(),
                           dck_e_.get(), dck_part_.get(), c0, dPartialTile_.get(), dck_q_.get(), dsp_p0_.get(),
                           dsp_n_.get(), dSplitCnt_.get());
    };
    if (h_.ck_wide[group]) {
        go(k_update<4, 1>);
    } else {
        if (occ == 4) go(k_update<1, 4>);
        else go(k_update<1, 1>);
    }
    return 1;
}

hipEvent_t KktDevice::next_event() {
    if (kev_used_ == kev_.size()) {
        hipEvent_t e;
        IPO_HIP_CHECK(hipEventCreate(&e));
        kev_.push_back(e);
    }
    return kev_[kev_used_++];
}

void KktDevice::ph_begin(hipStream_t s) {
    if (!timing_) return;
    mark_b_ = next_event();
    IPO_HIP_CHECK(hipEventRecord(mark_b_, s));
}

void KktDevice::ph_end(int phase, int launches, hipStream_t s) {
    if (!timing_) return;
    hipEvent_t e = next_event();
    IPO_HIP_CHECK(hipEventRecord(e, s));
    marks_.push_back({mark_b_, e, phase, launches});
}

void KktDevice::ph_collect() {
    for (const PhaseMark& mk : marks_) {
        float ms = 0;
        IPO_HIP_CHECK(hipEventElapsedTime(&ms, mk.b, mk.e));
        tm_.phase_ms[mk.phase] += ms;
        tm_.phase_launches[mk.phase] += mk.launches;
    }
    marks_.clear();
    kev_used_ = 0;
}

void KktDevice::launch_q_long(const double* v, double* out) {
    ipo::launch_q_long(q_long_n_, dQLongCols_.get(), dkQ_.get(), diQ_.get(), dQ_.get(), v, out, stream_);
}

void KktDevice::set_long_rows(int row0) {
    if (xch_ || row0 < 0 || row0 >= m_) return;
    long_row0_ = row0;
    dLongAx_.alloc(2 * static_cast<size_t>(m_ - row0));
}

void KktDevice::solve_multi(int R, const double* dE, const double* dD, double* const* dfy, double* const* dfx,
                            int* ok) {
    hipStream_t s = stream_;
    if (timing_) IPO_HIP_CHECK(hipEventRecord(ev0_, s));
    const int m = m_, n = n_, T = T_;
    const bool pre = take_prepass(R, dfy, dfx);
    if (!pre && R > 0) enqueue_pass_head(R, dfy, dfx, dPart_.get(), s);
    double maxbc[2] = {0.0, 0.0}, rs[2] = {HUGE_VAL, HUGE_VAL}, rs_old[2] = {HUGE_VAL, HUGE_VAL};
    int pass[2] = {0, 0};
    bool active[2] = {R > 0, R > 1};
    auto zv = [&](int r) { return dZ_.get() + (size_t)r * T; };
    auto dyv = [&](int r) { return dDy_.get() + (size_t)r * m; };
    auto dxv = [&](int r) { return dDx_.get() + (size_t)r * n; };
    auto ryv = [&](int r) { return dRy_.get() + (size_t)r * m; };
    auto rxv = [&](int r) { return dRx_.get() + (size_t)r * n; };
    int incons[2] = {0, 0};
    while (active[0] || active[1]) {
        const bool first = pass[0] + pass[1] == 0;
        if (!first) {
            PermJobs J{};
            int na = 0;
            for (int r = 0; r < R; r++)
                if (active[r]) {
                    J.fy[na] = ryv(r);
                    J.fx[na] = rxv(r);
                    J.z[na] = zv(r);
                    na++;
                }
            hipLaunchKernelGGL(k_perm_in2, dim3(ceil_div(T, NT), na), dim3(NT), 0, s, T, m, dperm_.get(), J,
                               dIncons_.get(), dScal_.get() + 4);
        }
        eps_cleared_ = true;
        const size_t fwd_first = first && pre ? static_cast<size_t>(h_.sweep.split) : 0;
        if (active[0] && active[1]) rawsolve(zv(0), 2, fwd_first);
        else rawsolve(zv(active[0] ? 0 : 1), 1, fwd_first);
        eps_cleared_ = false;
        int nq = 0;
        {
            PermJobs P{};
            ResJobs J{};
            const int mrow = xch_ ? m - nforced_ : long_row0_ >= 0 ? long_row0_ : m;
            for (int r = 0; r < R; r++) {
                if (!active[r]) continue;
                P.z[nq] = zv(r); P.dy[nq] = dyv(r); P.dx[nq] = dxv(r); P.mode[nq] = pass[r] == 0 ? 0 : 1;
                J.fy[nq] = dfy[r]; J.fx[nq] = dfx[r]; J.dy[nq] = dyv(r); J.dx[nq] = dxv(r);
                J.ry[nq] = ryv(r); J.rx[nq] = rxv(r);
                J.axl[nq] = xch_ ? dLinkAx_.get() + (size_t)r * nforced_
                                 : long_row0_ >= 0 ? dLongAx_.get() + (size_t)r * (m - long_row0_) : nullptr;
                J.qxl[nq] = q_long_n_ > 0 ? dLongQ_.get() + (size_t)r * m : nullptr;
                nq++;
            }
            hipLaunchKernelGGL(k_perm_out2, dim3(ceil_div(T, NT), nq), dim3(NT), 0, s, T, m, diperm_.get(), P);
            for (int q = 0; q < nq; q++) {
                double* axl = const_cast<double*>(J.axl[q]);
                if (xch_) {
                    launch_link_ax(mrow, m, dkAt_.get(), diAt_.get(), dAt_.get(), J.dx[q], axl, s);
                    xsum(axl, nforced_, RedOp::Sum);
                } else if (long_row0_ >= 0) {
                    launch_link_ax(mrow, m, dkAt_.get(), diAt_.get(), dAt_.get(), J.dx[q], axl, s);
                }
                if (q_long_n_ > 0) launch_q_long(J.dy[q], const_cast<double*>(J.qxl[q]));
            }
            hipLaunchKernelGGL(k_kkt_residual2, dim3(kRedBlocks, nq), dim3(kResThreads), 0, s, m, n, dkAt_.get(),
                               diAt_.get(), dAt_.get(), dkA_.get(), diA_.get(), dA_.get(), dE, dD, J, dPart_.get(), mrow,
                               dkQ_.get() ? dkQ_.get() : static_cast<const int*>(nullptr), diQ_.get(), dQ_.get(),
                               static_cast<double>(qmax_), q_long_min());
        }
        if (xch_) {
            hipLaunchKernelGGL(k_finish_reduce, dim3(1), dim3(kRedThreads), 0, s, dPart_.get(), nq, (1u << nq) - 1u,
                               dScal_.get());
            xsum(dScal_.get(), nq, RedOp::Max);
            hipLaunchKernelGGL(k_pack_ints, dim3(1), dim3(2), 0, s, dIncons_.get(), 2, dScal_.get() + 6);
        } else {
            hipLaunchKernelGGL(k_finish_reduce_pack, dim3(1), dim3(kRedThreads), 0, s, dPart_.get(), nq,
                               (1u << nq) - 1u, dScal_.get(), static_cast<const int*>(dIncons_.get()), 2,
                               dScal_.get() + 6);
        }
        IPO_HIP_CHECK(hipMemcpyAsync(hScal_, dScal_.get(), (pass[0] + pass[1] == 0 ? 8 + 2 * R : 7) * sizeof(double),
                                     hipMemcpyDeviceToHost, s));
        IPO_HIP_CHECK(hipStreamSynchronize(s));
        if (pass[0] + pass[1] == 0)
            for (int r = 0; r < R; r++)
                maxbc[r] = (hScal_[8 + 2 * r] > hScal_[8 + 2 * r + 1] ? hScal_[8 + 2 * r] : hScal_[8 + 2 * r + 1]) + 1;
        std::memcpy(hFlags_ + 2, hScal_ + 6, 2 * sizeof(int));
        int q = 0;
        for (int r = 0; r < R; r++) {
            if (!active[r]) continue;
            incons[r] = hFlags_[2 + q];
            rs_old[r] = rs[r];
            rs[r] = hScal_[q++];
            pass[r]++;
            active[r] = rs[r] > 1.0e-10 * maxbc[r] && rs[r] < rs_old[r] / 2;
        }
    }
    CopyOut co{};
    for (int r = 0; r < R; r++) {
        if (rs[r] > rs_old[r] && pass[r] > 1)
            hipLaunchKernelGGL(k_perm_out, dim3(ceil_div(T, NT)), dim3(NT), 0, s, T, m, diperm_.get(), zv(r), dyv(r),
                               dxv(r), 2);
        co.src[2 * r] = dyv(r); co.dst[2 * r] = dfy[r];
        co.src[2 * r + 1] = dxv(r); co.dst[2 * r + 1] = dfx[r];
    }
    co.m = m;
    co.n = n;
    co.R = R;
    if (R > 0 && m + n > 0) hipLaunchKernelGGL(k_copy_out, dim3(ceil_div(R * (m + n), NT)), dim3(NT), 0, s, co);
    if (timing_) {
        IPO_HIP_CHECK(hipEventRecord(ev1_, s));
        IPO_HIP_CHECK(hipStreamSynchronize(s));
        float ms = 0;
        IPO_HIP_CHECK(hipEventElapsedTime(&ms, ev0_, ev1_));
        tm_.solve_ms += ms;
    }
    tm_.solves += R;
    last_passes_ = pass[0] + pass[1];
    for (int r = 0; r < R; r++) ok[r] = incons[r] ? 0 : 1;
}

bool KktDevice::take_prepass(int R, double* const* dfy, double* const* dfx) {
    bool same = pre_state_ == kPreValid && !timing_ && pre_req_.R == R;
    for (int r = 0; same && r < R; r++) same = pre_req_.dfy[r] == dfy[r] && pre_req_.dfx[r] == dfx[r];
    if (!same) {
        drop_prepass();
        return false;
    }
    pre_state_ = kPreNone;
    pre_used_++;
    return true;
}

int KktDevice::solve(const double* dE, const double* dD, double* dfy, double* dfx) {
    int ok[1];
    solve_multi(1, dE, dD, &dfy, &dfx, ok);
    return ok[0];
}

int KktDevice::solve2(const double* dE, const double* dD, double* dfy1, double* dfx1, double* dfy2, double* dfx2) {
    double* fy[2] = {dfy1, dfy2};
    double* fx[2] = {dfx1, dfx2};
    int ok[2];
    solve_multi(2, dE, dD, fy, fx, ok);
    return ok[0] && ok[1];
}

void KktDevice::download_factor(double* lx, double* d, int* live) const {
    if (lx) dLx_.download(lx, plan_.lx_size, stream_);
    if (d) dDg_.download(d, T_, stream_);
    if (live) dLive_.download(live, T_, stream_);
    IPO_HIP_CHECK(hipStreamSynchronize(stream_));
}

}
```

### linear-programming-vanderbei_amd/csrc/kkt_knobs.h

```cpp
#pragma once
#include <algorithm>
#include <cstdlib>
#include <string>

#include "kkt_plan.h"

namespace ipo {

constexpr int kTailVisitBlocks = 4;
constexpr int kTailVisitLatest = 4;
constexpr int kLongQCol = 256;

struct KktKnobs {

    bool panel = true;
    bool merge_levels = true;
    bool sf = true;
    bool overlap = true;
    bool prepass = true;
    bool chain_lead = true;
    bool chain_pairs = false;
    bool tail_run = true;
    bool tail_winpub = true;
    bool visit_sched = true;
    bool visit_xcd = true;
    bool tail_repair = true;
    int tail_spec = 1;
    int sparse_dep = 1;
    int visits = -1;
    int gather_flat = 1;
    bool gather_quad = true;
    int small_leaves = -1;
    int panel_split = 768;
    int ax_blocks = 1;
    int ax_jds = -1;


    int visit_blocks = kTailVisitBlocks;
    int visit_latest = kTailVisitLatest;
    int visit_slabs = kVisitSlots / kSlab;
    int min_chunk = 64;
    int sf_width = -1;
    int update_xcd = 1024;
    int update_occ = 4;
    int dot_segmin = -1;
    int q_long = kLongQCol;


    bool setup_times = false;
    bool debug_redo = false;
    bool trace_full = false;
    std::string dump_dir;
    int gather_stamps = -1;
    double epsdiag_max = 0.0;
    double pivtol = 1.0e-17;
    std::string sf_stamps_file;

    bool deep_tree(int nlevels) const { return visits < 0 ? nlevels >= kVisitLevels : visits != 0; }

    static KktKnobs from_env() {
        const auto flag = [](const char* name, bool dflt) {
            const char* e = std::getenv(name);
            return e ? std::atoi(e) != 0 : dflt;
        };
        const auto num = [](const char* name, int dflt) {
            const char* e = std::getenv(name);
            return e ? std::atoi(e) : dflt;
        };
        const auto real = [](const char* name, double dflt) {
            const char* e = std::getenv(name);
            return e ? std::atof(e) : dflt;
        };
        const auto text = [](const char* name) {
            const char* e = std::getenv(name);
            return std::string(e ? e : "");
        };
        const auto set = [](const char* name) { return std::getenv(name) != nullptr; };
        KktKnobs k;
        k.panel = flag("IPO_HIP_PANEL", true);
        k.merge_levels = flag("IPO_HIP_MERGE_LEVELS", true);
        k.sf = flag("IPO_HIP_SF", true);
        k.overlap = flag("IPO_HIP_OVERLAP", true);
        k.prepass = flag("IPO_HIP_PREPASS", true);
        k.chain_lead = flag("IPO_HIP_CHAIN_LEAD", true);
        k.chain_pairs = flag("IPO_HIP_CHAIN_PAIRS", false);
        k.tail_run = flag("IPO_HIP_TAIL_RUN", true);
        k.tail_winpub = flag("IPO_HIP_TAIL_WINPUB", true);
        k.visit_sched = flag("IPO_HIP_VISIT_SCHED", true);
        k.visit_xcd = flag("IPO_HIP_VISIT_XCD", true);
        k.tail_repair = flag("IPO_HIP_TAIL_REPAIR", true);
        k.tail_spec = num("IPO_HIP_TAIL_SPEC", 1);
        k.sparse_dep = num("IPO_HIP_SPARSE_DEP", 1);
        if (set("IPO_HIP_VISITS")) k.visits = flag("IPO_HIP_VISITS", false);
        k.gather_flat = num("IPO_HIP_GATHER_FLAT", 1);
        k.gather_quad = flag("IPO_HIP_GATHER_QUAD", true);
        if (set("IPO_HIP_SMALL_LEAVES")) k.small_leaves = std::max(0, num("IPO_HIP_SMALL_LEAVES", 0));
        k.panel_split = std::max(0, num("IPO_HIP_PANEL_SPLIT", 768));
        k.ax_blocks = std::max(1, num("IPO_HIP_AX_BLOCKS", 1));
        if (set("IPO_HIP_AX_JDS")) k.ax_jds = flag("IPO_HIP_AX_JDS", false);
        k.visit_blocks = std::max(1, num("IPO_HIP_VISIT_BLOCKS", kTailVisitBlocks));
        k.visit_latest = std::max(1, num("IPO_HIP_VISIT_LATEST", kTailVisitLatest));
        if (set("IPO_HIP_VISIT_SLOTS")) k.visit_slabs = std::max(1, num("IPO_HIP_VISIT_SLOTS", 0) / kSlab);
        if (set("IPO_HIP_MIN_CHUNK")) k.min_chunk = std::max(kSlab, num("IPO_HIP_MIN_CHUNK", 0) / kSlab * kSlab);
        if (set("IPO_HIP_SF_WIDTH")) k.sf_width = std::max(1, num("IPO_HIP_SF_WIDTH", 0));
        k.update_xcd = std::max(0, num("IPO_HIP_UPDATE_XCD", 1024));
        k.update_occ = num("IPO_HIP_UPDATE_OCC", 4);
        if (set("IPO_HIP_DOT_SEGMIN")) k.dot_segmin = std::max(0, num("IPO_HIP_DOT_SEGMIN", 0));
        k.q_long = std::max(0, num("IPO_HIP_Q_LONG", kLongQCol));
        k.setup_times = set("IPO_HIP_SETUP_TIMES");
        k.debug_redo = set("IPO_HIP_DEBUG_REDO");
        k.trace_full = set("IPO_HIP_TRACE_FULL");
        k.dump_dir = text("IPO_HIP_DUMP_DIR");
        k.gather_stamps = num("IPO_HIP_GATHER_STAMPS", -1);
        k.epsdiag_max = real("IPO_HIP_EPSDIAG_MAX", 0.0);
        k.pivtol = real("IPO_HIP_PIVTOL", 1.0e-17);
        k.sf_stamps_file = text("IPO_SF_STAMPS_FILE");
        return k;
    }
};

}
```

### linear-programming-vanderbei_amd/csrc/kkt_schedule.cpp

```cpp
#include "kkt_schedule.h"

#include <algorithm>
#include <utility>

namespace ipo {

namespace {
int ceil_div(long a, long b) { return static_cast<int>((a + b - 1) / b); }
constexpr int PC = kPanelCols, TR = kTileRows;
int tail_gp(int nt, int t) { return std::max(1, (nt - t * PC + TR - 1) / TR - 1); }
}

KktPaths kkt_paths(const KktPlan& P, const KktKnobs& knobs) {
    KktPaths p;
    p.visits = knobs.deep_tree(P.nlevels);
    p.chain_lead = knobs.chain_lead && P.nt > 0 && P.ntb <= kChainMaxBlocks;
    p.tail_blocked = P.nt > 0 && P.ntb > kChainMaxBlocks;
    p.tail_run = knobs.tail_run && P.nt > 0 && P.ntb <= kTailSchedMaxBlocks;
    p.run_winpub = knobs.tail_winpub && p.tail_run;
    p.small_leaves = knobs.small_leaves < 0 ? kSmallLeafMinCount : knobs.small_leaves;
    p.sf_width = knobs.sf_width > 0 ? knobs.sf_width : P.lx_size < (int64_t(1) << 25) ? 300 : 64;
    return p;
}

// ... 233 lines not shown
        const int nc = P.col0[sp + 1] - P.col0[sp], h = nc + P.rowptr[sp + 1] - P.rowptr[sp];
        const int nrow = std::min(kTileRows, h - t * kTileRows);
        for (int q = 0; q < 4; q++) {
            const int qr = q & 1, qc = q >> 1;
            if (32 * qr >= nrow || 32 * qc >= nc || (t == 0 && qc > qr)) continue;
            cu.push_back(u); cb.push_back(kb); ce.push_back(ke); cp.push_back(-1 - q); cq.push_back(-1);
        }
    };
    auto group = [&](int u0, int u1, auto kbeg, auto kend, const std::vector<SchedInt3>* visits) {
        const long nck0 = static_cast<long>(cu.size());
        long sumk = 0, nun = 0;
        for (int u = u0; u < u1; u++) { sumk += kend(u) - kbeg(u); nun += kend(u) > kbeg(u); }
        const bool quad = quad_mode && visits && nun + static_cast<long>(visits->size()) <= kQuadMaxUnits;
        if (quad) {
            for (int u = u0; u < u1; u++)
                if (kend(u) > kbeg(u)) quadrants(u, kbeg(u), kend(u));
            for (const SchedInt3& v : *visits) quadrants(v.x, v.y, v.z);
            r.ck_wide.push_back(false);
            r.ck_kind.push_back(2);
            return;
        }
        long kmax = (sumk / wg_target + kSlab - 1) / kSlab * kSlab;
        kmax = std::max<long>(min_chunk, std::min<long>(kMaxChunkSlots, kmax));
        int np = 0, mx = 0;
        for (int u = u0; u < u1; u++) {
            const int kb = kbeg(u), ke = kend(u);
            if (ke == kb) continue;
            const int nch = static_cast<int>((ke - kb + kmax - 1) / kmax);
            mx = std::max(mx, nch);
            if (nch > 1) { su.push_back(u); sp0.push_back(np); sn.push_back(nch); }
            for (int j = 0; j < nch; j++) {
                cu.push_back(u);
                cb.push_back(kb + static_cast<int>(j * kmax));
                ce.push_back(std::min<int>(ke, kb + static_cast<int>((j + 1) * kmax)));
                cp.push_back(nch > 1 ? np++ : -1);
                cq.push_back(nch > 1 ? static_cast<int>(su.size()) - 1 : -1);
            }
        }
        if (visits)
            for (const SchedInt3& v : *visits) {
                cu.push_back(v.x); cb.push_back(v.y); ce.push_back(v.z); cp.push_back(-1); cq.push_back(-1);
            }
        max_part = std::max<size_t>(max_part, np);
        r.ck_wide.push_back(mx >= 4 && static_cast<long>(cu.size()) - nck0 <= 512);
        r.ck_kind.push_back(quad ? 2 : (flat_mode == 2 || (flat_mode == 1 && paths.visits)) &&
                                               static_cast<long>(cu.size()) - nck0 <= kFlatMaxChunks ? 1 : 0);
    };
    const std::vector<int>& kp = P.kslot_ptr;
    for (int l = 0; l < P.nlevels; l++) {
        if (l == 0) { r.ck_wide.push_back(false); r.ck_kind.push_back(0); }
        else if (paths.visits)
            group(P.unit_level_ptr[l], P.unit_level_ptr[l + 1], [&](int u) { return vs.late_b[u]; },
                  [&](int u) { return vs.kptr[u + 1]; }, &vs.vis[l]);
        else
            group(P.unit_level_ptr[l], P.unit_level_ptr[l + 1], [&](int u) { return kp[u]; },
                  [&](int u) { return kp[u + 1]; }, nullptr);
        r.ck_ptr[l + 1] = static_cast<int>(cu.size());
        r.sp_ptr[l + 1] = static_cast<int>(su.size());
    }
    const std::vector<int>& tp = P.tail_kslot_ptr;
    if (P.nt > 0)
        group(0, P.ntb * (P.ntb + 1) / 2, [&](int u) { return tp[u]; }, [&](int u) { return tp[u + 1]; },
              nullptr);
    else { r.ck_wide.push_back(false); r.ck_kind.push_back(0); }
    r.ck_ptr[P.nlevels + 1] = static_cast<int>(cu.size());
    r.sp_ptr[P.nlevels + 1] = static_cast<int>(su.size());
    r.split_cnt = std::max<size_t>(1, su.size());
    r.partial_tiles = std::max<size_t>(1, max_part);
    return r;
}

int sweep_launches(const std::vector<SweepStep>& steps) {
    int n = 0;
    for (const SweepStep& st : steps) n += st.kind == kSwChunked ? 2 : 1;
    return n;
}

int sweep_split(const std::vector<SweepStep>& fwd) {
    for (size_t i = 0; i + 1 < fwd.size(); i++)
        if (fwd[i].kind == kSwTailGather) return fwd[i + 1].kind == kSwTailLead ? static_cast<int>(i) + 1 : 0;
    return 0;
}

SweepSteps build_sweep_steps(const KktPlan& P, const KktKnobs& knobs, const KktPaths& paths, const SolveChunks& ch,
                             const SweepOrder& order, const SyncFreePlan& sf, bool blocked) {
    SweepSteps r;
    auto level = [&](int l, std::vector<SweepStep>& out) {
        const int q0 = P.level_ptr[l], q1 = P.level_ptr[l + 1];
        const int cb = ch.chunk_ptr[l], ce = ch.chunk_ptr[l + 1];
        if (ce > cb) { out.push_back({kSwChunked, q0, q1 - q0, cb, ce - cb}); return; }
        const int nl = blocked ? 0 : order.leaf_cnt[l], n8 = blocked ? 0 : order.leaf8_cnt[l];
        if (n8 > 0) out.push_back({kSwLeaf8, q0, n8, 0, 0});
        if (nl > n8 && q1 - q0 > nl && knobs.merge_levels) {
            out.push_back({kSwMerged, q0 + n8, nl - n8, q1 - q0 - nl, 0});
        } else {
            if (nl > n8) out.push_back({kSwLeaf, q0 + n8, nl - n8, 0, 0});
            if (q1 - q0 > nl) out.push_back({kSwPlain, q0 + nl, q1 - q0 - nl, 0, 0});
        }
    };
    const bool range = !blocked && sf.range(P);
    const int top = blocked ? P.nlevels : sf.sf_level;
    const int pre_cols = static_cast<int>(sf.pre_col.size());
    for (int l = 0; l < top; l++) level(l, r.fwd);
    if (range) {
        if (pre_cols > 0) r.fwd.push_back({kSwPre, 0, pre_cols, 0, 0});
        r.fwd.push_back({kSwSyncFree, 0, static_cast<int>(sf.items_f.size()), pre_cols > 0 || sf.late_lists, 0});
    }
    if (P.nt > 0) {
        r.fwd.push_back({kSwTailGather, 0, 0, 0, 0});
        if (blocked) {
            for (int kb = 0; kb < P.ntb; kb++) r.fwd.push_back({kSwTailBlock, 0, 0, kb, 0});
            r.bwd.push_back({kSwTailDscale, 0, 0, 0, 0});
            for (int kb = P.ntb - 1; kb >= 0; kb--) r.bwd.push_back({kSwTailBlock, 0, 0, kb, 0});
        } else {
            r.fwd.push_back({paths.chain_lead ? kSwTailLead : kSwTailChain, 0, 0, 0, 0});
            r.bwd.push_back({knobs.chain_pairs ? kSwTailPair : kSwTailChain, 0, 0, 0, 0});
        }
    }
    if (range) r.bwd.push_back({kSwSyncFree, 0, static_cast<int>(sf.items_b.size()), 0, 0});
    for (int l = top - 1; l >= 0; l--) level(l, r.bwd);
    r.split = sweep_split(r.fwd);
    return r;
}

WorkCounts count_work(const KktPlan& P, const KktKnobs& knobs, const SweepSteps& sweep) {
    WorkCounts w;
    w.fwd_launches = sweep_launches(sweep.fwd);
    w.bwd_launches = sweep_launches(sweep.bwd);
    double gb = 0;
    auto tasks_bytes = [&](const std::vector<TailTask>& ts) {
        for (const TailTask& t : ts) {
            const double ncd = P.col0[t.src + 1] - P.col0[t.src];
            const double nr = __builtin_popcountll(t.rmask), ncl = __builtin_popcountll(t.cmask);
            gb += 8.0 * ncd * (nr + ncl);
        }
    };
    tasks_bytes(P.utasks);
    tasks_bytes(P.tail_tasks);
    double db = 0, tb = 0, sb = 0;
    for (int sp = 0; sp < P.nsup; sp++) {
        const double nc = P.col0[sp + 1] - P.col0[sp], hb = P.rowptr[sp + 1] - P.rowptr[sp];
        db += 8.0 * 1.5 * nc * nc;
        tb += 16.0 * hb * nc;
        gb += 16.0 * (nc + hb) * nc;
    }
    const double sdb = db, stb = tb;
    for (int kb = 0; kb < P.ntb; kb++) {
        const double nc = std::min(kPanelCols, P.nt - kb * kPanelCols), below = P.nt - kb * kPanelCols - nc;
        db += 8.0 * 1.5 * nc * nc;
        tb += 16.0 * below * nc;
        const double nb = P.ntb - kb - 1;
        sb += (nb * (nb + 1) / 2) * (16.0 * kTileRows * kTileRows + 16.0 * kTileRows * nc);
    }
    gb += 16.0 * 0.5 * P.nt * P.nt;
    w.bytes[kPhGather] = gb;
    w.bytes[kPhDiag] = db;
    w.bytes[kPhTrsm] = tb;
    w.bytes[kPhSyrk] = sb;
    w.flops[kPhGather] = P.narth_gather;
    if (knobs.panel) {
        w.flops[kPhDiag] = P.narth_panel; w.bytes[kPhDiag] = sdb + stb;
        w.flops[kPhTrsm] = w.bytes[kPhTrsm] = 0;
        w.flops[kPhSyrk] = w.bytes[kPhSyrk] = 0;
        w.flops[kPhTail] = P.narth_tail;
        w.bytes[kPhTail] = 16.0 * (static_cast<double>(P.lnz_tail) + P.nt);
    } else {
        w.flops[kPhDiag] = P.narth_panel;
        w.flops[kPhTrsm] = 0;
        w.flops[kPhSyrk] = P.narth_tail;
    }
    for (int ph : {kPhForward, kPhBackward}) {
        w.flops[ph] = 2.0 * static_cast<double>(P.lnz) + 0.5 * P.T;
        w.bytes[ph] = 12.0 * static_cast<double>(P.lnz) + 16.0 * P.T;
    }
    return w;
}

std::vector<TaskSrc> build_task_src(const KktPlan& P, const std::vector<TailTask>& ts) {
    std::vector<TaskSrc> v(ts.size());
    for (size_t t = 0; t < ts.size(); t++) {
        const int d = ts[t].src, ncd = P.col0[d + 1] - P.col0[d];
        v[t].colbase = P.off[d] + ncd;
        v[t].hd = ncd + (P.rowptr[d + 1] - P.rowptr[d]);
        v[t].cd0 = P.col0[d];
    }
    return v;
}

std::vector<SlotRec> build_slot_records(const KktPlan& P, const std::vector<int>& kslot,
                                        const std::vector<TailTask>& ts) {
    std::vector<SlotRec> v(kslot.size());
    for (size_t i = 0; i < kslot.size(); i++) {
        const int sl = kslot[i];
        SlotRec& r = v[i];
        if (sl < 0) { r.rmask = r.cmask = 0; r.roff = 0; r.cdelta = 0; r.dk = 0; continue; }
        const TailTask& t = ts[sl >> 6];
        const int kl = sl & 63, d = t.src, ncd = P.col0[d + 1] - P.col0[d];
        const int64_t hd = ncd + (P.rowptr[d + 1] - P.rowptr[d]);
        r.rmask = t.rmask;
        r.cmask = t.cmask;
        r.roff = P.off[d] + ncd + kl * hd + t.rbase;
        r.cdelta = t.cbase - t.rbase;
        r.dk = P.col0[d] + kl;
    }
// ... 185 lines not shown
```

### linear-programming-vanderbei_amd/csrc/kkt_schedule.h

```cpp
#pragma once
#include <cstddef>
#include <cstdint>
#include <vector>

#include "kkt_knobs.h"
#include "kkt_plan.h"

namespace ipo {

constexpr int kSmallLeaf = 8;
constexpr int kSmallLeafMinCount = 32768;
constexpr int kChunkRows = 128;
constexpr int kChainMaxBlocks = 200;
constexpr int kTailSchedMaxBlocks = 255;

enum KktPhase { kPhGather = 0, kPhDiag, kPhTrsm, kPhSyrk, kPhForward, kPhBackward, kPhTail, kNumPhases };

struct SchedInt2 { int x, y; };
struct SchedInt3 { int x, y, z; };
struct SchedUint2 { unsigned x, y; };

struct KktPaths {
    bool visits = false;
    bool chain_lead = false;
    bool tail_blocked = false;
    bool tail_run = false;
    bool run_winpub = false;
    int small_leaves = 0;
    int sf_width = 0;
};
KktPaths kkt_paths(const KktPlan& P, const KktKnobs& knobs);

enum SweepKind {
    kSwChunked = 0,
    kSwPlain,
    kSwLeaf8,
    kSwMerged,
    kSwLeaf,
    kSwPre,
    kSwSyncFree,
    kSwTailGather,
    kSwTailLead,
    kSwTailChain,
    kSwTailPair,
    kSwTailBlock,
    kSwTailDscale,
};
struct SweepStep { int kind, q0, n, a, b; };
struct SweepSteps {
    std::vector<SweepStep> fwd, bwd;
    int split = 0;
};
int sweep_split(const std::vector<SweepStep>& fwd);
int sweep_launches(const std::vector<SweepStep>& steps);

struct KktLaunch {
    KktPaths paths;
    std::vector<int> fu_ptr;
    std::vector<int> small_ptr;
    std::vector<char> split_level;
    std::vector<int> small1_cnt;
    SweepSteps sweep;
    size_t partial_stride = 1;
    int sf_level = 0;
    size_t ybuf_stride = 1, zpad_stride = 1;
    std::vector<int> ck_ptr;
    std::vector<int> ck_kind;
    std::vector<char> ck_wide;
    std::vector<int> visit_ptr;
    std::vector<int> run_ptr;
};

struct PanelUnits {
    std::vector<int> fu_sup, fu_j;
    std::vector<int> small_sups;
    std::vector<int> fu_ptr, small_ptr, small1_cnt;
    std::vector<char> split_level;
};
PanelUnits build_panel_units(const KktPlan& P, const KktKnobs& knobs, const KktPaths& paths);

struct SolveChunks {
    std::vector<int> chunk_sup, chunk_r0;
    std::vector<int> sup_chunk0;
    std::vector<int> chunk_ptr;
    size_t partial_stride = 1;
};
SolveChunks build_solve_chunks(const KktPlan& P);

struct SweepOrder {
    std::vector<int> sweep_sups;
    std::vector<int> leaf_cnt, leaf8_cnt;
};
SweepOrder build_sweep_order(const KktPlan& P, const KktPaths& paths, const SolveChunks& ch);

struct SyncFreePlan {
    int sf_level = 0;
    std::vector<int> ybase;
    std::vector<int> yrow_idx;
    std::vector<int> zbase, zpi, need, par;
    std::vector<SchedInt2> items_f, items_b;
    size_t ybuf_stride = 1, zpad_stride = 1;
    bool late_lists = false;
    std::vector<int> ylate_ptr, ylate_idx, pre_col, pre_ptr, pre_idx;
    bool range(const KktPlan& P) const { return sf_level < P.nlevels; }
};
SyncFreePlan build_sync_free_plan(const KktPlan& P, const KktKnobs& knobs, const KktPaths& paths,
                                  const SolveChunks& ch);

struct VisitSlots {
    std::vector<int> kslot, kptr, late_b;
    std::vector<std::vector<SchedInt3>> vis;
};
VisitSlots build_visit_slots(const KktPlan& P, const KktKnobs& knobs, const KktPaths& paths);

struct GatherChunks {
    std::vector<int> ck_u, ck_b, ck_e, ck_part;
    std::vector<int> ck_q;
    std::vector<int> sp_u, sp_p0, sp_n;
    std::vector<int> ck_ptr, sp_ptr, ck_kind;
    std::vector<char> ck_wide;
    size_t split_cnt = 1;
    size_t partial_tiles = 1;
};
GatherChunks build_gather_chunks(const KktPlan& P, const KktKnobs& knobs, const KktPaths& paths,
                                 const VisitSlots& vs);

SweepSteps build_sweep_steps(const KktPlan& P, const KktKnobs& knobs, const KktPaths& paths, const SolveChunks& ch,
                             const SweepOrder& order, const SyncFreePlan& sf, bool blocked);

struct WorkCounts {
    int fwd_launches = 0, bwd_launches = 0;
    double flops[kNumPhases] = {}, bytes[kNumPhases] = {};
};
WorkCounts count_work(const KktPlan& P, const KktKnobs& knobs, const SweepSteps& sweep);

std::vector<TaskSrc> build_task_src(const KktPlan& P, const std::vector<TailTask>& ts);
std::vector<SlotRec> build_slot_records(const KktPlan& P, const std::vector<int>& kslot,
                                        const std::vector<TailTask>& ts);


constexpr inline int visit_hi(int t, int c, int K) { return c - 1 - K * (c - 1 - t); }

int tail_visit_tiles(int ntb, int t, int K);
std::vector<unsigned> tail_visit_schedule(int ntb, int nt, int K, int cap, bool xcd, std::vector<int>& ptr);
std::vector<SchedUint2> tail_run_schedule(int ntb, int nt, int K, int L, int cap, std::vector<int>& ptr);
void tail_visit_work(int ntb, int nt, int K, double& flops, double& bytes);

struct TailSchedule {
    std::vector<unsigned> visit_list;
    std::vector<int> visit_ptr;
    std::vector<SchedUint2> run_items;
    std::vector<int> run_ptr;
};
TailSchedule build_tail_schedule(const KktPlan& P, const KktKnobs& knobs, const KktPaths& paths, int cus);

struct KktSchedule {
    KktPaths paths;
    PanelUnits panels;
    SolveChunks chunks;
    SweepOrder order;
    SyncFreePlan sf;
    VisitSlots visits;
    GatherChunks gather;
    SweepSteps sweep;
    WorkCounts work;
    std::vector<TaskSrc> usrc, tsrc;
    std::vector<SlotRec> slot_rec, tail_slot_rec;
    TailSchedule tail;
};
KktSchedule build_kkt_schedule(const KktPlan& P, const KktKnobs& knobs, int cus);

}
```

### linear-programming-vanderbei_amd/csrc/kkt_sweep.hip

```cpp
#include <hip/hip_runtime.h>

#include <algorithm>
#include <array>
#include <climits>
#include <cstdio>
#include <initializer_list>
#include <map>
#include <stdexcept>
#include <string>
#include <vector>

#include "dev_common.h"
#include "kkt_device.h"
#include "kkt_kernels.h"

namespace ipo {

namespace {

__device__ __forceinline__ int opaque_lane() {
    int lane = threadIdx.x & 63;
    asm volatile("" : "+v"(lane));
    return lane;
}
// ... 1048 lines not shown
#pragma unroll
            for (int r = 0; r < R; r++) zb[r][lane] = zj[r];
        }
        __syncthreads();
#pragma unroll
        for (int r = 0; r < R; r++) {
            const double zr = lane < nr ? zb[r][lane] : 0.0;
#pragma unroll
            for (int q = 0; q < 16; q++) {
                acch[r][q] += th[q] * zr;
                accl[r][q] += tl[q] * zr;
            }
        }
        __syncthreads();
    }
    double tlh[16];
    {
        const int rr = kh + (lane < nch ? lane : 0);
        const double* __restrict__ col = tv.S + rr + (size_t)(kl + (nql > 0 ? kq : 0)) * nt;
#pragma unroll
        for (int q = 0; q < 16; q++) tlh[q] = col[(size_t)min(q, max(nql, 1) - 1) * nt];
    }
    double* red = lds_pad;
    if (hi < ntb - 1) {
        if (nqh > 0) colsum_put<R>(red, acch, kq, nqh, lane);
        __syncthreads();
        if (tid < R * PC && tid % PC < nch) xs[tid / PC][tid % PC] = colsum_tree(red, tid / PC, tid % PC);
        __syncthreads();
    }
    if (wv == 0) {
        double zr[R];
#pragma unroll
        for (int r = 0; r < R; r++) zr[r] = lane < nch ? zdh[r] - (hi < ntb - 1 ? xs[r][lane] : 0.0) : 0.0;
        tri_upper<R>(zr, Ls[0], lv[0], nch, eps, badh);
        if (lane < nch) {
#pragma unroll
            for (int r = 0; r < R; r++) {
                gran_put(gran + (((size_t)hi * R + r) * 64 + lane) * 2, epoch, zr[r]);
                V.z[r * V.zs + tc + kh + lane] = zr[r];
            }
        }
#pragma unroll
        for (int r = 0; r < R; r++) zb[r][lane] = zr[r];
        flag_bad<R>(p, badh);
    }
    if (!haslo) return;
    __syncthreads();
#pragma unroll
    for (int r = 0; r < R; r++) {
        const double zr = lane < nch ? zb[r][lane] : 0.0;
#pragma unroll
        for (int q = 0; q < 16; q++) accl[r][q] += tlh[q] * zr;
    }
    if (nql > 0) colsum_put<R>(red, accl, kq, nql, lane);
    __syncthreads();
    if (tid < R * PC && tid % PC < ncl) xs[tid / PC][tid % PC] = colsum_tree(red, tid / PC, tid % PC);
    __syncthreads();
    if (wv == 0) {
        double zr[R];
#pragma unroll
        for (int r = 0; r < R; r++) zr[r] = lane < ncl ? zdl[r] - xs[r][lane] : 0.0;
        tri_upper<R>(zr, Ls[1], lv[1], ncl, eps, badl);
        if (lane < ncl) {
#pragma unroll
            for (int r = 0; r < R; r++) {
                gran_put(gran + (((size_t)lo * R + r) * 64 + lane) * 2, epoch, zr[r]);
                V.z[r * V.zs + tc + kl + lane] = zr[r];
            }
        }
        flag_bad<R>(p, badl);
    }
}

constexpr int kLeadBlocks = 2;
#ifdef IPO_LEAD_STAMPS
__device__ double g_lead_stats[8][4];
#define LEAD_T(v) const long long v = wall_clock64()
#else
#define LEAD_T(v) do {} while (0)
#endif
__device__ __forceinline__ __amdgpu_buffer_rsrc_t tail_rsrc(const double* S) {
    return __builtin_amdgcn_make_buffer_rsrc(const_cast<double*>(S), 0, 0x7fffffff, 0x00020000);
}
__device__ __forceinline__ double buf_ld(__amdgpu_buffer_rsrc_t rs, int voff, int soff) {
    typedef int i32x2 __attribute__((ext_vector_type(2)));
    const i32x2 v = __builtin_amdgcn_raw_buffer_load_b64(rs, voff, soff, 0);
    return __builtin_bit_cast(double, v);
}
constexpr int kLeadNT = 448;
constexpr int kHelpBatch = 4;
__device__ __forceinline__ gran_t* part_slot(gran_t* pg, int i, int R, int r, int g, int lane) {
    return pg + (((((size_t)i * R + r) * 4 + g) * 64) + lane) * 2;
}
__device__ __forceinline__ void lds_sync() {
    __builtin_amdgcn_fence(__ATOMIC_RELEASE, "workgroup", "local");
    __builtin_amdgcn_s_barrier();
    __builtin_amdgcn_fence(__ATOMIC_ACQUIRE, "workgroup", "local");
}

template <int R>
__global__ void __launch_bounds__(kLeadNT)
k_tail_fwd_lead(PlanView p, TailView tv, SweepVecs V, const double* __restrict__ epsp, gran_t* __restrict__ gran,
                gran_t* __restrict__ pgran, unsigned epoch, int* __restrict__ ticket, int tbase) {
    extern __shared__ double lds[];
    constexpr int K = kLeadBlocks;
    const int nt = tv.nt, tc = tv.tc, ntb = tv.ntb;
    const int tid = threadIdx.x, lane = tid & 63, wv = __builtin_amdgcn_readfirstlane(tid >> 6);
    const int g = wv <= 3 ? wv - 1 : wv - 2;
    const int pl = g * 64 + lane;
    __shared__ int role_sh;
    if (tid == 0) role_sh = __hip_atomic_fetch_add(ticket, 1, __ATOMIC_RELAXED, __HIP_MEMORY_SCOPE_AGENT) - tbase;
    __syncthreads();
    const int role = role_sh;
    if (wv == 4 || (wv == 6 && (R == 1 || role > 0))) return;
    if (role > 0) {
        const int i = role + K, k0 = i * PC, nc = min(PC, nt - k0), jend = i - K;
        double* zb = lds;
        const __amdgpu_buffer_rsrc_t rs = tail_rsrc(tv.S);
        const int nt8 = nt * 8, g16 = __builtin_amdgcn_readfirstlane(g * 16);
        const int voff = (k0 + (lane < nc ? lane : 0)) * 8;
        double acc[R];
#pragma unroll
        for (int r = 0; r < R; r++) acc[r] = 0.0;
        for (int j0 = 0; j0 < jend; j0 += kHelpBatch) {
            double t[kHelpBatch][16];
            if (wv > 0) {
#pragma unroll
                for (int b = 0; b < kHelpBatch; b++) {
                    const int s0 = (min(j0 + b, jend - 1) * PC + g16) * nt8;
#pragma unroll
                    for (int q = 0; q < 16; q++) t[b][q] = buf_ld(rs, voff, s0 + q * nt8);
                }
            } else {
#pragma unroll
                for (int b = 0; b < kHelpBatch; b++) {
                    if (j0 + b < jend) {
                        double zj[R];
                        gran_wait<R>(gran + (size_t)(j0 + b) * R * 128, epoch, lane, PC, zj);
#pragma unroll
                        for (int r = 0; r < R; r++) zb[(b * R + r) * PC + lane] = zj[r];
                    }
                }
            }
            lds_sync();
            if (wv > 0) {
#pragma unroll
                for (int b = 0; b < kHelpBatch; b++) {
                    if (j0 + b < jend) {
#pragma unroll
                        for (int q = 0; q < 16; q++) {
#pragma unroll
                            for (int r = 0; r < R; r++) acc[r] += t[b][q] * zb[(b * R + r) * PC + g * 16 + q];
                        }
                    }
                }
            }
            lds_sync();
        }
        if (wv > 0) {
#pragma unroll
            for (int r = 0; r < R; r++) gran_put(part_slot(pgran, i, R, r, g, lane), epoch, acc[r]);
        }
        return;
    }
    double(*Ls)[PC][PC + 1] = reinterpret_cast<double(*)[PC][PC + 1]>(lds);
    double* zh = lds + 2 * PC * (PC + 1);
    double* red = zh + K * R * PC;
    int* lv = reinterpret_cast<int*>(red + R * 4 * 64);
    if (wv == 0 || wv == 6) {
        const int rs = wv == 0 ? 0 : 1;
        double eps[1] = {epsp[rs]}, zown[1];
        int bad[1] = {};
        zown[0] = lane < min(PC, nt) ? V.z[rs * V.zs + tc + lane] : 0.0;
#ifdef IPO_LEAD_STAMPS
        long long sa = 0, st = 0, sb = 0;
#endif
        lds_sync();
        for (int i = 0; i < ntb; i++) {
            LEAD_T(t0);
            const int k0 = i * PC, nc = min(PC, nt - k0);
            double znext;
            const int k1 = k0 + PC, nc1 = i + 1 < ntb ? min(PC, nt - k1) : 0;
            znext = lane < nc1 ? V.z[rs * V.zs + tc + k1 + lane] : 0.0;
            lds_sync();
            LEAD_T(t1);
            double zr[1];
            {
                const double* rd = red + rs * 4 * 64 + lane;
                zr[0] = lane < nc ? zown[0] - (((rd[0] + rd[64]) + rd[128]) + rd[192]) : 0.0;
            }
            tri_lower<1, true>(zr, Ls[i & 1], lv + (i & 1) * PC, nc, eps, bad);
            LEAD_T(t2);
            if (lane < nc) {
                gran_put(gran + (((size_t)i * R + rs) * 64 + lane) * 2, epoch, zr[0]);
                V.z[rs * V.zs + tc + k0 + lane] = zr[0];
            }
            zh[((i % K) * R + rs) * PC + lane] = lane < nc ? zr[0] : 0.0;
            zown[0] = znext;
            lds_sync();
#ifdef IPO_LEAD_STAMPS
            LEAD_T(t3);
            sa += t1 - t0; st += t2 - t1; sb += t3 - t2;
#endif
        }
#ifdef IPO_LEAD_STAMPS
        if (lane == 0 && wv == 0) {
            g_lead_stats[0][0] = sa * 0.01 / ntb; g_lead_stats[0][1] = st * 0.01 / ntb;
            g_lead_stats[0][2] = sb * 0.01 / ntb;
        }
#endif
        if (bad[0]) atomicOr(&p.incons[rs], 1);
        return;
    }
    const __amdgpu_buffer_rsrc_t rs = tail_rsrc(tv.S);
    const int nt8 = nt * 8, g16 = __builtin_amdgcn_readfirstlane(g * 16);
    auto load_tiles = [&](int i, double(&t)[K][16]) {
        const int k0 = i * PC, nc = min(PC, nt - k0);
        const int voff = (k0 + (lane < nc ? lane : 0)) * 8;
#pragma unroll
        for (int b = 0; b < K; b++) {
            const int s0 = (max(i - K + b, 0) * PC + g16) * nt8;
#pragma unroll
            for (int q = 0; q < 16; q++) t[b][q] = buf_ld(rs, voff, s0 + q * nt8);
        }
    };
    auto l11_load = [&](int i, double(&t)[16], int& lvv) {
        const int k0 = i * PC, nc = min(PC, nt - k0);
        const int voff = (k0 + lane) * 8;
#pragma unroll
        for (int q = 0; q < 16; q++) {
            const int r = g + 4 * q;
            const bool ok = r < nc && lane < r;
            t[q] = buf_ld(rs, ok ? voff : 0, min(k0 + r, nt - 1) * nt8);
        }
        lvv = p.live[tc + k0 + min(pl, nc - 1)];
    };
    auto l11_store = [&](int i, const double(&t)[16], int lvv) {
        const int nc = min(PC, nt - i * PC);
#pragma unroll
        for (int q = 0; q < 16; q++) {
            const int r = g + 4 * q;
            Ls[i & 1][r][lane] = r < nc && lane < r ? t[q] : 0.0;
        }
        if (pl < nc) lv[(i & 1) * PC + pl] = lvv;
    };
    unsigned long long praw[R][2];
    auto part_load = [&](int i) {
#pragma unroll
        for (int r = 0; r < R; r++) {
            const gran_t* q = part_slot(pgran, i, R, r, g, lane);
            praw[r][0] = __hip_atomic_load(const_cast<gran_t*>(q), __ATOMIC_RELAXED, __HIP_MEMORY_SCOPE_AGENT);
            praw[r][1] = __hip_atomic_load(const_cast<gran_t*>(q + 1), __ATOMIC_RELAXED, __HIP_MEMORY_SCOPE_AGENT);
        }
    };
    double pre[R];
#pragma unroll
    for (int r = 0; r < R; r++) pre[r] = 0.0;
    double tA[K][16], tB[K][16], lA[16], lB[16];
    int vA, vB;
#ifdef IPO_LEAD_STAMPS
    long long pw = 0, p3 = 0, p4 = 0;
    int polls = 0;
#endif
    l11_load(0, lA, vA);
    l11_store(0, lA, vA);
    load_tiles(min(1, ntb - 1), tB);
    l11_load(min(1, ntb - 1), lB, vB);
    part_load(min(1, ntb - 1));
    lds_sync();
    auto step = [&](int i, double(&cur)[K][16], double(&nxt)[K][16], double(&lcur)[16], int& vcur,
                    double(&lnxt)[16], int& vnxt) {
        double acc[R];
#pragma unroll
        for (int r = 0; r < R; r++) acc[r] = pre[r];
        if (i >= 1) {
            const double* z = zh + ((i - 1) % K) * R * PC + g * 16;
#pragma unroll
            for (int q = 0; q < 16; q++) {
#pragma unroll
                for (int r = 0; r < R; r++) acc[r] += cur[K - 1][q] * z[r * PC + q];
            }
        }
#pragma unroll
        for (int r = 0; r < R; r++) red[(r * 4 + g) * 64 + lane] = acc[r];
        lds_sync();
        LEAD_T(u0);
        if (i + 1 < ntb) {
            l11_store(i + 1, lnxt, vnxt);
            if (i + 1 > K) {
                for (;;) {
                    bool ok = true;
#pragma unroll
                    for (int r = 0; r < R; r++) ok &= (praw[r][0] >> 32) == epoch && (praw[r][1] >> 32) == epoch;
                    if (__all(ok)) break;
#ifdef IPO_LEAD_STAMPS
                    polls++;
#endif
                    __builtin_amdgcn_s_sleep(IPO_POLL_SLEEP);
                    part_load(i + 1);
                }
                LEAD_T(u1);
#ifdef IPO_LEAD_STAMPS
                pw += u1 - u0;
#endif
#pragma unroll
                for (int r = 0; r < R; r++)
                    pre[r] = __longlong_as_double(static_cast<long long>(((praw[r][1] & 0xffffffffull) << 32) |
                                                                         (praw[r][0] & 0xffffffffull)));
            } else {
#pragma unroll
                for (int r = 0; r < R; r++) pre[r] = 0.0;
            }
#pragma unroll
            for (int b = 0; b < K - 1; b++) {
                const int j = i + 1 - K + b;
                if (j >= 0) {
                    const double* z = zh + (j % K) * R * PC + g * 16;
#pragma unroll
                    for (int q = 0; q < 16; q++) {
#pragma unroll
                        for (int r = 0; r < R; r++) pre[r] += nxt[b][q] * z[r * PC + q];
                    }
                }
                __builtin_amdgcn_sched_barrier(0);
            }
        }
        LEAD_T(u2);
        const int i2 = min(i + 2, ntb - 1);
        load_tiles(i2, cur);
        l11_load(i2, lcur, vcur);
        part_load(i2);
        LEAD_T(u3);
#ifdef IPO_LEAD_STAMPS
        p3 += u2 - u0; p4 += u3 - u2;
#endif
        lds_sync();
    };
    int i = 0;
    for (; i + 1 < ntb; i += 2) {
        step(i, tA, tB, lA, vA, lB, vB);
        step(i + 1, tB, tA, lB, vB, lA, vA);
    }
    if (i < ntb) step(i, tA, tB, lA, vA, lB, vB);
#ifdef IPO_LEAD_STAMPS
    if (lane == 0) {
        g_lead_stats[wv][0] = pw * 0.01 / ntb; g_lead_stats[wv][1] = polls;
        g_lead_stats[wv][2] = p3 * 0.01 / ntb; g_lead_stats[wv][3] = p4 * 0.01 / ntb;
    }
#endif
}

constexpr int kSfIdx = static_cast<int>(kChainLds / sizeof(int));

struct SfView {
    const int2* items;
    int nitems;
    int* cnt;
    int* flag;
    const int* need;
    const int* parent;
    const int* zbase;
    const int* zpi;
    double* zpad;
    size_t zps;
    int epoch;
    int* ticket;
    int tbase;
};

__device__ __forceinline__ int sf_draw(const SfView& sf) {
    return __hip_atomic_fetch_add(sf.ticket, 1, __ATOMIC_RELAXED, __HIP_MEMORY_SCOPE_AGENT) - sf.tbase;
}
__device__ __forceinline__ void sf_next(int* tk, int nxt) {
    if (threadIdx.x == 0) *tk = nxt;
    __syncthreads();
}

__device__ __forceinline__ void sf_arrive_next(int* c, int* tk, int nxt) {
    asm volatile("s_waitcnt vmcnt(0)" ::: "memory");
    if (threadIdx.x == 0) *tk = nxt;
    __syncthreads();
    if (threadIdx.x == 0) __hip_atomic_fetch_add(c, 1, __ATOMIC_RELAXED, __HIP_MEMORY_SCOPE_AGENT);
}
__device__ __forceinline__ void sf_publish_next(int* flags, int i, int epoch, int* tk, int nxt) {
    asm volatile("s_waitcnt vmcnt(0)" ::: "memory");
    if (threadIdx.x == 0) *tk = nxt;
    __syncthreads();
    if (threadIdx.x == 0) __hip_atomic_store(flags + i, epoch, __ATOMIC_RELAXED, __HIP_MEMORY_SCOPE_AGENT);
}


template <int R>
__global__ void __launch_bounds__(NT)
k_fwd_pre(int ncols, const int* __restrict__ col, const int* __restrict__ eptr, const int* __restrict__ eidx,
          SweepVecs V) {
    const int j = blockIdx.x * NT + threadIdx.x;
    if (j >= ncols) return;
    const int c = col[j];
    double acc[R];
#pragma unroll
    for (int r = 0; r < R; r++) acc[r] = 0.0;
    int e = eptr[j];
    const int e1 = eptr[j + 1];
    for (; e + 7 < e1; e += 8) {
        int ix[8];
#pragma unroll
        for (int u = 0; u < 8; u++) ix[u] = eidx[e + u];
#pragma unroll
        for (int r = 0; r < R; r++) {
            double yv[8];
#pragma unroll
            for (int u = 0; u < 8; u++) yv[u] = V.y[r * V.ys + ix[u]];
#pragma unroll
            for (int u = 0; u < 8; u++) acc[r] += yv[u];
        }
    }
    for (; e < e1; e++) {
        const int i0 = eidx[e];
#pragma unroll
        for (int r = 0; r < R; r++) acc[r] += V.y[r * V.ys + i0];
    }
#pragma unroll
    for (int r = 0; r < R; r++) V.z[r * V.zs + c] -= acc[r];
}
// ... 287 lines not shown
            if (lane < nc)
                for (int c = wv; c < nch; c += 4) {
#pragma unroll
                    for (int r = 0; r < R; r++) x[r] += sc1_load(part + r * ps + (size_t)(cf + c) * PC + lane);
                }
#pragma unroll
            for (int r = 0; r < R; r++) xs[r][wv][lane] = x[r];
        } else if (pre) {
            double acc[R][16];
#pragma unroll
            for (int r = 0; r < R; r++)
#pragma unroll
                for (int q = 0; q < 16; q++) acc[r][q] = 0.0;
            double zi[kPre][R];
#pragma unroll
            for (int u = 0; u < kPre; u++)
                if (lane + 64 * u < hb) sf_zrow<R>(sf, V, rip[u], pip[u], zi[u]);
#pragma unroll
            for (int u = 0; u < kPre; u++)
                if (lane + 64 * u < hb) {
#pragma unroll
                    for (int q = 0; q < 16; q++)
                        if (q < nq) {
#pragma unroll
                            for (int r = 0; r < R; r++) acc[r][q] += tp[u][q] * zi[u][r];
                        }
                }
            colsum_put<R>(red, acc, kq, nq, lane);
        } else if (nq > 0) {
            double acc[R][16];
#pragma unroll
            for (int r = 0; r < R; r++)
#pragma unroll
                for (int q = 0; q < 16; q++) acc[r][q] = 0.0;
            for (int i = lane; i < hb; i += 64) {
                double zi[R];
                sf_zrow<R>(sf, V, rows[i], sf.zpi[rows[i]], zi);
                const double* __restrict__ col = panel + nc + i + (size_t)kq * h;
                double t[16];
#pragma unroll
                for (int q = 0; q < 16; q++) t[q] = col[(size_t)min(q, nq - 1) * h];
#pragma unroll
                for (int q = 0; q < 16; q++)
                    if (q < nq) {
#pragma unroll
                        for (int r = 0; r < R; r++) acc[r][q] += t[q] * zi[r];
                    }
            }
            colsum_put<R>(red, acc, kq, nq, lane);
        }
        __syncthreads();
        if (code != -2) {
            if (tid < R * PC && tid % PC < nc) xs[tid / PC][0][tid % PC] = colsum_tree(red, tid / PC, tid % PC);
            __syncthreads();
        }
        if (wv < R) bwd_sf_solve<R>(p, sf, V, s, c0, nc, code == -2, zown, lvo, dgo, eps, Ls, lv, xs, wv);
        sf_publish_next(sf.flag, s, sf.epoch, slot, nxt);
    }
}

__global__ void k_scale_scalar(double* e, int n, double f) { if (static_cast<int>(threadIdx.x) < n) e[threadIdx.x] *= f; }

}

void KktDevice::raise_sweep_lds(bool sync_free) {
    struct Lds { const void* f; int bytes; };
    auto raise = [](std::initializer_list<Lds> table) {
        for (const Lds& e : table)
            IPO_HIP_CHECK(hipFuncSetAttribute(e.f, hipFuncAttributeMaxDynamicSharedMemorySize, e.bytes));
    };
    if (sync_free && h_.sf_level < plan_.nlevels)
        raise({{reinterpret_cast<const void*>(&k_fwd_sf<1>), kChainLds},
               {reinterpret_cast<const void*>(&k_fwd_sf<2>), kChainLds},
               {reinterpret_cast<const void*>(&k_bwd_sf<1>), kChainLds},
               {reinterpret_cast<const void*>(&k_bwd_sf<2>), kChainLds}});
    if (!sync_free && plan_.nt > 0 && plan_.ntb <= kChainMaxBlocks)
        raise({{reinterpret_cast<const void*>(&k_tail_fwd_chain<1>), kChainLds},
               {reinterpret_cast<const void*>(&k_tail_fwd_chain<2>), kChainLds},
               {reinterpret_cast<const void*>(&k_tail_bwd_chain<1>), kChainLds},
               {reinterpret_cast<const void*>(&k_tail_bwd_chain<2>), kChainLds},
               {reinterpret_cast<const void*>(&k_tail_bwd_pair<1>), kPairBwdLds},
               {reinterpret_cast<const void*>(&k_tail_bwd_pair<2>), kPairBwdLds},
               {reinterpret_cast<const void*>(&k_tail_fwd_lead<1>), kChainLds},
               {reinterpret_cast<const void*>(&k_tail_fwd_lead<2>), kChainLds}});
}

void KktDevice::dump_sf_stamps() const {
#ifdef IPO_SF_STAMPS
    const std::vector<SchedInt2>& items = h_sf_items_f_;
    const KktPlan& P = plan_;
    const std::string& file = knobs_.sf_stamps_file;
    if (items.empty()) return;
    std::vector<long long> st((size_t)(1 << 15) * 10);
    if (hipMemcpyFromSymbol(st.data(), HIP_SYMBOL(g_sfst), st.size() * sizeof(long long)) != hipSuccess) return;
    const int n = std::min<int>(items.size(), 1 << 15);
    long long t0 = LLONG_MAX;
    for (int i = 0; i < n; i++) t0 = std::min(t0, st[i * 10]);
    std::map<int, std::array<double, 7>> lv;
    for (int i = 0; i < n; i++) {
        const long long* x = &st[i * 10];
        auto& a = lv[P.level[items[i].x]];
        a[0] += 1; a[1] += x[1] - x[0]; a[2] += x[2] - x[1]; a[3] += x[3] - x[2]; a[4] = std::max<double>(a[4], x[4] - t0);
        a[5] += x[4] - x[3];
    }
    if (!file.empty()) {
        if (FILE* fo = std::fopen(file.c_str(), "w")) {
            for (int i = 0; i < n; i++) {
                const long long* x = &st[i * 10];
                std::fprintf(fo, "%d %d %d %d %lld %lld %lld %lld %lld %lld %lld %lld %lld\n", items[i].x, items[i].y,
                             P.level[items[i].x], P.parent[items[i].x], x[0] - t0, x[1] - t0, x[2] - t0, x[3] - t0,
                             x[4] - t0, x[5] - t0, x[6], x[7] - t0, x[8] - t0);
            }
            std::fclose(fo);
        }
    }
    std::fprintf(stderr, "sf forward: level items wait diag rest handoff end(us)\n");
    for (auto& [l, a] : lv)
        std::fprintf(stderr, "  %3d %4.0f %7.2f %7.2f %7.2f %6.2f %8.1f\n", l, a[0], a[1] / a[0] / 100, a[2] / a[0] / 100,
                     a[3] / a[0] / 100, a[5] / a[0] / 100, a[4] / 100);
#endif
}

template <int R>
void KktDevice::sweep(double* dz, const double* epsp, size_t fwd_first) {
    hipStream_t s = stream_;
    if (timing_) IPO_HIP_CHECK(hipEventRecord(ev2_, s));
    ph_begin(s);
    const int nf = run_sweep_steps<R>(h_.sweep.fwd, true, dz, epsp, fwd_first);
    ph_end(kPhForward, nf, s);
    ph_begin(s);
    const int nb = run_sweep_steps<R>(h_.sweep.bwd, false, dz, epsp);
    ph_end(kPhBackward, nb, s);
    IPO_HIP_CHECK(hipGetLastError());
    if (timing_) {
        IPO_HIP_CHECK(hipEventRecord(ev3_, s));
        IPO_HIP_CHECK(hipEventSynchronize(ev3_));
        float ms = 0;
        IPO_HIP_CHECK(hipEventElapsedTime(&ms, ev2_, ev3_));
        tm_.sweep_ms += ms;
        ph_collect();
        tm_.phase_count[kPhForward]++;
        tm_.phase_count[kPhBackward]++;
    }
}

template <int R>
int KktDevice::run_sweep_steps(const std::vector<SweepStep>& steps, bool forward, double* dz, const double* epsp,
                               size_t first, size_t last, hipStream_t s) {
    if (!s) s = stream_;
    const PlanView pv = plan_view();
    const TailView tv = tail_view();
    const SweepVecs V{dz, static_cast<size_t>(T_), dYbuf_.get(), h_.ybuf_stride};
    const size_t ps = h_.partial_stride;
    const int nt = plan_.nt;
    int launched = 0;
    for (size_t i = first; i < std::min(last, steps.size()); i++) {
        const SweepStep& step = steps[i];
        const int q0 = step.q0, n = step.n;
        switch (step.kind) {
        case kSwChunked: {
            const int cb = step.a, nch = step.b;
            if (forward) {
                hipLaunchKernelGGL(k_fwd_diag<R>, dim3(n), dim3(NT), 0, s, pv, dsweep_sups_.get(), q0, dyrow_ptr_.get(),
                                   dyrow_idx_.get(), V, epsp);
                hipLaunchKernelGGL(k_fwd_gemv<R>, dim3(nch), dim3(NT), 0, s, pv, dchunk_sup_.get(), dchunk_r0_.get(),
                                   cb, V);
            } else {
                hipLaunchKernelGGL(k_bwd_partial<R>, dim3(nch), dim3(NT), 0, s, pv, dchunk_sup_.get(), dchunk_r0_.get(),
                                   cb, V, dPartial_.get(), ps);
                hipLaunchKernelGGL(k_bwd_finish<R>, dim3(n), dim3(NT), 0, s, pv, dsweep_sups_.get(), q0,
                                   dsup_chunk0_.get(), dPartial_.get(), ps, V, epsp);
            }
            launched++;
            break;
        }
        case kSwPlain:
            if (forward)
                hipLaunchKernelGGL(k_forward<R>, dim3(n), dim3(NT), 0, s, pv, dsweep_sups_.get(), q0, dyrow_ptr_.get(),
                                   dyrow_idx_.get(), V, epsp);
            else
                hipLaunchKernelGGL(k_backward<R>, dim3(n), dim3(NT), 0, s, pv, dsweep_sups_.get(), q0, V, epsp);
            break;
        case kSwLeaf8:
            if (forward)
                hipLaunchKernelGGL(k_fwd_leaf8<R>, dim3(ceil_div(n, NT / kSmallLeaf)), dim3(NT), 0, s, pv,
                                   dsweep_sups_.get(), q0, n, dyrow_ptr_.get(), dyrow_idx_.get(), V, epsp);
            else
                hipLaunchKernelGGL(k_bwd_leaf8<R>, dim3(ceil_div(n, NT / kSmallLeaf)), dim3(NT), 0, s, pv,
                                   dsweep_sups_.get(), q0, n, V, epsp);
            break;
        case kSwMerged: {
            const int nlb = ceil_div(n, NT / 64);
            if (forward)
                hipLaunchKernelGGL(k_fwd_level<R>, dim3(nlb + step.a), dim3(NT), 0, s, pv, dsweep_sups_.get(), q0, n,
                                   nlb, dyrow_ptr_.get(), dyrow_idx_.get(), V, epsp);
            else
                hipLaunchKernelGGL(k_bwd_level<R>, dim3(nlb + step.a), dim3(NT), 0, s, pv, dsweep_sups_.get(), q0, n,
                                   nlb, V, epsp);
            break;
        }
        case kSwLeaf:
            if (forward)
                hipLaunchKernelGGL(k_fwd_leaf<R>, dim3(ceil_div(n, NT / 64)), dim3(NT), 0, s, pv, dsweep_sups_.get(),
                                   q0, n, dyrow_ptr_.get(), dyrow_idx_.get(), V, epsp);
            else
                hipLaunchKernelGGL(k_bwd_leaf<R>, dim3(ceil_div(n, NT / 64)), dim3(NT), 0, s, pv, dsweep_sups_.get(),
                                   q0, n, V, epsp);
            break;
        case kSwPre:
            hipLaunchKernelGGL(k_fwd_pre<R>, dim3(ceil_div(n, NT)), dim3(NT), 0, s, n, dpre_col_.get(), dpre_ptr_.get(),
                               dpre_idx_.get(), V);
            break;
        case kSwSyncFree:
            if (forward) {
                const SfView sf{dsf_items_f_.get(), n, dsf_fcnt_.get(), dsf_fflag_.get(), dsf_need_.get(),
                                dsf_par_.get(), dsf_zbase_.get(), dsf_zpi_.get(), dZpad_.get(), h_.zpad_stride,
                                ++sf_fwd_epoch_, dsf_ticket_.get(), sf_tbase(0, n, s)};
                const bool pre = step.a != 0;
                hipLaunchKernelGGL(k_fwd_sf<R>, dim3(std::min(sf_grid_, n)), dim3(NT), kChainLds, s, pv, sf,
                                   pre ? dylate_ptr_.get() : dyrow_ptr_.get(),
                                   pre ? dylate_idx_.get() : dyrow_idx_.get(), dchunk_r0_.get(), V, epsp);
            } else {
                const SfView sf{dsf_items_b_.get(), n, dsf_bcnt_.get(), dsf_bflag_.get(), dsf_need_.get(),
                                dsf_par_.get(), dsf_zbase_.get(), dsf_zpi_.get(), dZpad_.get(), h_.zpad_stride,
                                ++sf_bwd_epoch_, dsf_ticket_.get() + 1, sf_tbase(1, n, s)};
                hipLaunchKernelGGL(k_bwd_sf<R>, dim3(std::min(sf_grid_, n)), dim3(NT), kChainLds, s, pv, sf,
                                   dchunk_r0_.get(), dsup_chunk0_.get(), dPartial_.get(), ps, V, epsp);
            }
            break;
        case kSwTailGather:
            tail_rhs_begin(dz, R);
            hipLaunchKernelGGL(k_tail_gather<R>, dim3(ceil_div(nt, 4)), dim3(NT), 0, s, tv, dyrow_ptr_.get(),
                               dyrow_idx_.get(), V);
            tail_rhs_end(dz, R);
            break;
        case kSwTailLead: {
            const int grid = 1 + std::max(0, plan_.ntb - 1 - kLeadBlocks);
            if (lead_ticket_next_ + grid > (1LL << 30)) {
                IPO_HIP_CHECK(hipMemsetAsync(dlead_ticket_.get(), 0, sizeof(int), s));
                lead_ticket_next_ = 0;
            }
            const int tb = static_cast<int>(lead_ticket_next_);
            lead_ticket_next_ += grid;
            hipLaunchKernelGGL(k_tail_fwd_lead<R>, dim3(grid), dim3(kLeadNT), kChainLds, s, pv, tv, V, epsp,
                               dChainGran_.get(), dChainGran_.get() + static_cast<size_t>(plan_.ntb) * 2 * 128,
                               ++chain_epoch_, dlead_ticket_.get(), tb);
#ifdef IPO_LEAD_STAMPS
            if (chain_epoch_ % 64 == 41) {
                double st[8][4];
                IPO_HIP_CHECK(hipStreamSynchronize(s));
                IPO_HIP_CHECK(hipMemcpyFromSymbol(st, HIP_SYMBOL(g_lead_stats), sizeof(st)));
                std::fprintf(stderr, "lead R %d ntb %d per step us: solver wait-A %.3f tri %.3f wait-B %.3f\n", R,
                             plan_.ntb, st[0][0], st[0][1], st[0][2]);
                for (int w = 1; w <= 4; w++)
                    std::fprintf(stderr, "  wave %d: partial wait %.3f (%g polls) phase3 %.3f loads %.3f\n", w,
                                 st[w][0], st[w][1], st[w][2], st[w][3]);
            }
#endif
            break;
        }
        case kSwTailChain:
            if (forward)
                hipLaunchKernelGGL(k_tail_fwd_chain<R>, dim3(plan_.ntb), dim3(NT), kChainLds, s, pv, tv, V, epsp,
                                   dChainGran_.get(), ++chain_epoch_);
            else
                hipLaunchKernelGGL(k_tail_bwd_chain<R>, dim3(plan_.ntb), dim3(NT), kChainLds, s, pv, tv, V, epsp,
                                   dChainGran_.get(), ++chain_epoch_);
            break;
        case kSwTailPair:
            hipLaunchKernelGGL(k_tail_bwd_pair<R>, dim3((plan_.ntb + 1) / 2), dim3(NT), kPairBwdLds, s, pv, tv, V, epsp,
                               dChainGran_.get(), ++chain_epoch_);
            break;
        case kSwTailBlock: {
            const int kb = step.a;
            if (forward) {
                const int below = nt - std::min(nt, (kb + 1) * kPanelCols);
                hipLaunchKernelGGL(k_tail_fwd, dim3(std::max(1, ceil_div(below, 64))), dim3(NT), 0, s, pv, tv, kb, dz,
                                   epsp);
            } else {
                const int left = kb * kPanelCols;
                hipLaunchKernelGGL(k_tail_bwd, dim3(std::max(1, ceil_div(left, 64))), dim3(NT), 0, s, pv, tv, kb, dz,
                                   epsp);
            }
            break;
        }
        case kSwTailDscale:
            hipLaunchKernelGGL(k_tail_dscale, dim3(ceil_div(nt, NT)), dim3(NT), 0, s, pv, tv, dz, epsp);
            break;
        default:
            throw std::logic_error("sweep: unknown step kind");
        }
        launched++;
    }
    return launched;
}

void KktDevice::run_prepass_steps(int R, hipStream_t q) {
    double* epsp = dScal_.get() + 4;
    const size_t split = static_cast<size_t>(h_.sweep.split);
    if (R == 2) run_sweep_steps<2>(h_.sweep.fwd, true, dZ_.get(), epsp, 0, split, q);
    else run_sweep_steps<1>(h_.sweep.fwd, true, dZ_.get(), epsp, 0, split, q);
}

int KktDevice::sf_tbase(int d, int nitems, hipStream_t s) {
    const long long draw = static_cast<long long>(nitems) + std::min(sf_grid_, nitems);
    if (sf_ticket_next_[d] + draw > (1LL << 30)) {
        IPO_HIP_CHECK(hipMemsetAsync(dsf_ticket_.get() + d, 0, sizeof(int), s));
        sf_ticket_next_[d] = 0;
    }
    const int base = static_cast<int>(sf_ticket_next_[d]);
    sf_ticket_next_[d] += draw;
    return base;
}

void KktDevice::tail_rhs_begin(double* dz, int R) {
    if (!shard_minor()) return;
    for (int r = 0; r < R; r++)
        IPO_HIP_CHECK(hipMemsetAsync(dz + (size_t)r * T_ + plan_.tail_c0, 0, sizeof(double) * plan_.nt, stream_));
}
void KktDevice::tail_rhs_end(double* dz, int R) {
    for (int r = 0; r < R; r++) xsum(dz + (size_t)r * T_ + plan_.tail_c0, plan_.nt, RedOp::Sum);
}

void KktDevice::rawsolve(double* dz, int R, size_t fwd_first) {
    hipStream_t s = stream_;
    double* epsp = dScal_.get() + 4;
    if (ndep_ > 0) {
        RedJobs j{};
        j.nj = R;
        for (int r = 0; r < R; r++) { j.a[r] = dz + (size_t)r * T_; j.b[r] = nullptr; j.len[r] = n_; j.op[r] = 1; }
        launch_reduce(j, dPart_.get(), epsp, s);
        hipLaunchKernelGGL(k_scale_scalar, dim3(1), dim3(64), 0, s, epsp, R, 1.0e-6);
        xsum(epsp, R, RedOp::Max);
    } else if (!eps_cleared_) {
        IPO_HIP_CHECK(hipMemsetAsync(epsp, 0, R * sizeof(double), s));
    }
    if (R == 2 && !h_.paths.tail_blocked) {
        sweep<2>(dz, epsp, fwd_first);
    } else {
        for (int r = 0; r < R; r++) sweep<1>(dz + (size_t)r * T_, epsp + r, fwd_first);
    }
    tm_.rawsolves += R;
}

}
```

Before: 298.8 iterations/s.

## Overlap forward tail-lead solve with tail factorization via per-column completion counters

Adds a trailing variant of the forward tail lead kernel that runs on the prepass stream alongside the tail-run factorization. It waits on new per-column completion counters (cdone) that the panel workers signal, and bails out if the factorization aborts. When the prepass is taken, the solve then resumes after the lead step instead of after the split. The goal is to hide the forward triangular solve of the dense tail behind the factorization. In exchange it adds polling, sc1 loads and extra concurrent blocks that compete with the factorization for compute units.

```diff
diff --git a/include/ipo_hip.h b/include/ipo_hip.h
--- a/include/ipo_hip.h
+++ b/include/ipo_hip.h
@@ -135,6 +135,8 @@
 
 int ipo_hip_tail_run_schedule(int nt, int K, int L, int cap, unsigned *items, int max_items, int *ptr);
 
+int ipo_hip_lead_col_targets(int nt, int *out, int cap);
+
 long ipo_hip_kkt_schedule(int m, int n, const int *kA, const int *iA, int nforced, int cus, const char *name, int *out,
                           long cap);
 
diff --git a/linear-programming-vanderbei_amd/csrc/capi.cpp b/linear-programming-vanderbei_amd/csrc/capi.cpp
--- a/linear-programming-vanderbei_amd/csrc/capi.cpp
+++ b/linear-programming-vanderbei_amd/csrc/capi.cpp
@@ -839,6 +839,7 @@
     if (name == "sweep.fwd") return steps(S.sweep.fwd);
     if (name == "sweep.bwd") return steps(S.sweep.bwd);
     if (name == "sweep.split") return {S.sweep.split};
+    if (name == "sweep.lead_end") return {S.sweep.lead_end};
     if (name == "sweep.fwd_blocked" || name == "sweep.bwd_blocked") {
         const ipo::SweepSteps b = ipo::build_sweep_steps(P, knobs, S.paths, S.chunks, S.order, S.sf, true);
         return steps(name == "sweep.fwd_blocked" ? b.fwd : b.bwd);
@@ -896,6 +897,18 @@
             }
         if (ptr) std::copy(pv.begin(), pv.end(), ptr);
         return n;
+    } catch (const std::exception& e) {
+        set_err(e.what());
+        return -1;
+    }
+}
+
+int ipo_hip_lead_col_targets(int nt, int* out, int cap) {
+    try {
+        if (nt <= 0) throw std::invalid_argument("lead_col_targets: bad arguments");
+        const int ntb = (nt + ipo::kPanelCols - 1) / ipo::kPanelCols;
+        for (int t = 0; out && t < std::min(ntb, cap); t++) out[t] = ipo::lead_col_target(nt, t);
+        return ntb;
     } catch (const std::exception& e) {
         set_err(e.what());
         return -1;
diff --git a/linear-programming-vanderbei_amd/csrc/kkt_dense.hip b/linear-programming-vanderbei_amd/csrc/kkt_dense.hip
--- a/linear-programming-vanderbei_amd/csrc/kkt_dense.hip
+++ b/linear-programming-vanderbei_amd/csrc/kkt_dense.hip
@@ -983,7 +983,12 @@
             if (c < nc) st_h<SC>(panel + row + (size_t)c * ld, a[q]);
         }
     }
-    if (j == 0 && tid < nc) { st_h<SC>(p.dg + c0 + tid, dv[tid]); p.live[c0 + tid] = DEP ? S.lv[tid] != 0 : 1; }
+    if (j == 0 && tid < nc) {
+        st_h<SC>(p.dg + c0 + tid, dv[tid]);
+        const int lvk = DEP ? S.lv[tid] != 0 : 1;
+        if constexpr (SC) __hip_atomic_store(p.live + c0 + tid, lvk, __ATOMIC_RELAXED, __HIP_MEMORY_SCOPE_AGENT);
+        else p.live[c0 + tid] = lvk;
+    }
     post(false);
     if (!fu_sup && pre && j == 0 && !h1 && lane < nc && (lane >> 4) == w) st_h<SC>(p.dscale + c0 + lane, dsc_pre);
     if (j != 0) return false;
@@ -1269,7 +1274,11 @@
             if (tr && threadIdx.x == 0) tr[1] = __builtin_amdgcn_s_memrealtime();
             return go;
         };
-        auto post = [&](bool bailed) { run_signal(rc.pdone + t, bailed ? 1 + kRunBail : 1); };
+        bool held = false;
+        auto post = [&](bool bailed) {
+            run_signal(rc.pdone + t, bailed ? 1 + kRunBail : 1);
+            held = !bailed;
+        };
         if (tr && threadIdx.x == 0 && t == 0) tr[1] = __builtin_amdgcn_s_memrealtime();
         PanelLds& S = *reinterpret_cast<PanelLds*>(lds);
         const RunPub rp{rc.pub, rc.wflag, rc.wflag, rc.pread, rc.t0, rc.epoch, vd, vt, q, &sh_ok};
@@ -1279,6 +1288,7 @@
             panel_w_body<true, true>(p, nullptr, nullptr, 0, tv, t, j, S, nullptr, t > 0, nullptr, t, tv.dep, NoWait{},
                                      post, rp);
         }
+        if (rc.cdone && held) run_signal(rc.cdone + t);
     } else {
         const int bi = rec.x & 255, c = (rec.x >> 8) & 255, b0 = (rec.x >> 16) & 255, b1 = rec.x >> 24;
         int* vs = rc.vseq + bi * ntb + c;
diff --git a/linear-programming-vanderbei_amd/csrc/kkt_device.h b/linear-programming-vanderbei_amd/csrc/kkt_device.h
--- a/linear-programming-vanderbei_amd/csrc/kkt_device.h
+++ b/linear-programming-vanderbei_amd/csrc/kkt_device.h
@@ -34,6 +34,7 @@
     int* ticket;
     int* pdone;
     int* vseq;
+    int* cdone = nullptr;
     double* pub = nullptr;
     int* wflag = nullptr;
     int* pread = nullptr;
@@ -230,12 +231,22 @@
     void run_prepass_steps(int R, hipStream_t q);
     void enqueue_pass_head(int R, double* const* dfy, double* const* dfx, double* part, hipStream_t s);
     bool take_prepass(int R, double* const* dfy, double* const* dfx);
-    void drop_prepass() { if (pre_state_ != kPreNone) { pre_state_ = kPreNone; pre_discarded_++; } }
+    void drop_prepass() {
+        if (pre_state_ != kPreNone) { pre_state_ = kPreNone; pre_discarded_++; lead_discarded_ += pre_lead_; }
+        pre_lead_ = false;
+        lead_pending_ = 0;
+    }
     enum { kPreNone = 0, kPreEnqueued, kPreValid };
     int pre_state_ = kPreNone;
     PrePass pre_req_;
     hipEvent_t ev_pre_fork_ = nullptr, ev_pre_done_ = nullptr;
     long pre_used_ = 0, pre_discarded_ = 0;
+    int lead_pending_ = 0;
+    bool pre_lead_ = false;
+    hipEvent_t ev_run_reset_ = nullptr;
+    long lead_used_ = 0, lead_discarded_ = 0;
+    void launch_lead_trail(int R, hipStream_t s, bool beside);
+    int* run_cdone() { return drun_cnt_.get() + 1 + plan_.ntb + static_cast<size_t>(plan_.ntb) * plan_.ntb + plan_.ntb; }
     DevBuf<double> dPrePart_;
     void enqueue_levels(const PlanView& pv, const TailView& tv, bool fused, hipStream_t s, const PrePass* pre);
     bool finish_pass(bool fused);
diff --git a/linear-programming-vanderbei_amd/csrc/kkt_device.hip b/linear-programming-vanderbei_amd/csrc/kkt_device.hip
--- a/linear-programming-vanderbei_amd/csrc/kkt_device.hip
+++ b/linear-programming-vanderbei_amd/csrc/kkt_device.hip
@@ -947,7 +947,7 @@
             static_assert(sizeof(SchedUint2) == sizeof(uint2), "SchedUint2 is uploaded as uint2");
             drun_items_.upload(reinterpret_cast<const uint2*>(ts.run_items.data()), ts.run_items.size(), s);
             h_.run_ptr = std::move(ts.run_ptr);
-            drun_cnt_.alloc(1 + plan_.ntb + static_cast<size_t>(plan_.ntb) * plan_.ntb + plan_.ntb);
+            drun_cnt_.alloc(1 + plan_.ntb + static_cast<size_t>(plan_.ntb) * plan_.ntb + plan_.ntb + plan_.ntb + 1);
             if (h_.paths.run_winpub) {
                 drun_pub_.alloc(2 * static_cast<size_t>(plan_.ntb) * 4 * kTailPubWin);
                 drun_wflag_.alloc(static_cast<size_t>(plan_.ntb) * plan_.ntb * 4);
@@ -989,6 +989,7 @@
     IPO_HIP_CHECK(hipEventCreate(&ev3_));
     IPO_HIP_CHECK(hipEventCreateWithFlags(&ev_pre_fork_, hipEventDisableTiming));
     IPO_HIP_CHECK(hipEventCreateWithFlags(&ev_pre_done_, hipEventDisableTiming));
+    IPO_HIP_CHECK(hipEventCreateWithFlags(&ev_run_reset_, hipEventDisableTiming));
     IPO_HIP_CHECK(hipStreamSynchronize(s));
 }
 
@@ -1044,8 +1045,10 @@
                              "k_panel_s %ld; tail block columns repaired %ld in %ld rounds\n", tm_.factors,
                      tm_.panel_redos, tm_.redo_where[0], tm_.redo_where[1], tm_.redo_where[2], tm_.redo_where[3],
                      tm_.tail_repairs, tm_.tail_dep_rounds);
-    if (knobs_.debug_redo)
+    if (knobs_.debug_redo) {
         std::fprintf(stderr, "kkt: forward pre-passes used %ld, discarded %ld\n", pre_used_, pre_discarded_);
+        std::fprintf(stderr, "kkt: trailing leads used %ld, discarded %ld\n", lead_used_, lead_discarded_);
+    }
     if (hScal_) (void)hipHostFree(hScal_);
     if (hFlags_) (void)hipHostFree(hFlags_);
     if (ev0_) (void)hipEventDestroy(ev0_);
@@ -1054,6 +1057,7 @@
     if (ev3_) (void)hipEventDestroy(ev3_);
     if (ev_pre_fork_) (void)hipEventDestroy(ev_pre_fork_);
     if (ev_pre_done_) (void)hipEventDestroy(ev_pre_done_);
+    if (ev_run_reset_) (void)hipEventDestroy(ev_run_reset_);
     for (hipEvent_t e : kev_) (void)hipEventDestroy(e);
 }
 
@@ -1248,6 +1252,8 @@
     IPO_HIP_CHECK(hipEventRecord(ev_pre_done_, q));
     pre_req_ = pre;
     pre_state_ = kPreEnqueued;
+    pre_lead_ = false;
+    lead_pending_ = h_.sweep.lead_end > 0 ? knobs_.lead_trail_mode(plan_.ntb) : 0;
 }
 
 void KktDevice::enqueue_levels(const PlanView& pv, const TailView& tv, bool fused, hipStream_t s, const PrePass* pre) {
@@ -1356,6 +1362,7 @@
     rc.ticket = drun_cnt_.get();
     rc.pdone = drun_cnt_.get() + 1;
     rc.vseq = drun_cnt_.get() + 1 + plan_.ntb;
+    rc.cdone = run_cdone();
     if (h_.paths.run_winpub) {
         if (run_epoch_ == INT_MAX) {
             IPO_HIP_CHECK(hipMemsetAsync(drun_wflag_.get(), 0, drun_wflag_.bytes(), s));
@@ -1367,9 +1374,19 @@
         if (!reset) IPO_HIP_CHECK(hipMemsetAsync(rc.pread + t0, 0, (plan_.ntb - t0) * sizeof(int), s));
         rc.epoch = ++run_epoch_;
     }
+    if (lead_pending_ == 2) IPO_HIP_CHECK(hipEventRecord(ev_run_reset_, s));
     ph_begin(s);
     launch_tail_run(pv, tail_view(), rc, s);
     ph_end(kPhTail, rc.n > 0, s);
+    if (lead_pending_) {
+        hipStream_t q = lead_pending_ == 2 ? pre_req_.stream : s;
+        if (lead_pending_ == 2) IPO_HIP_CHECK(hipStreamWaitEvent(q, ev_run_reset_, 0));
+        else IPO_HIP_CHECK(hipStreamWaitEvent(q, ev_pre_done_, 0));
+        launch_lead_trail(pre_req_.R, q, lead_pending_ == 2);
+        if (lead_pending_ == 2) IPO_HIP_CHECK(hipEventRecord(ev_pre_done_, q));
+        pre_lead_ = true;
+        lead_pending_ = 0;
+    }
 }
 
 void KktDevice::repair_tail() {
@@ -1501,6 +1518,7 @@
     hipStream_t s = stream_;
     if (timing_) IPO_HIP_CHECK(hipEventRecord(ev0_, s));
     const int m = m_, n = n_, T = T_;
+    const bool pre_lead = pre_lead_;
     const bool pre = take_prepass(R, dfy, dfx);
     if (!pre && R > 0) enqueue_pass_head(R, dfy, dfx, dPart_.get(), s);
     double maxbc[2] = {0.0, 0.0}, rs[2] = {HUGE_VAL, HUGE_VAL}, rs_old[2] = {HUGE_VAL, HUGE_VAL};
@@ -1528,7 +1546,7 @@
                                dIncons_.get(), dScal_.get() + 4);
         }
         eps_cleared_ = true;
-        const size_t fwd_first = first && pre ? static_cast<size_t>(h_.sweep.split) : 0;
+        const size_t fwd_first = first && pre ? static_cast<size_t>(pre_lead ? h_.sweep.lead_end : h_.sweep.split) : 0;
         if (active[0] && active[1]) rawsolve(zv(0), 2, fwd_first);
         else rawsolve(zv(active[0] ? 0 : 1), 1, fwd_first);
         eps_cleared_ = false;
@@ -1623,6 +1641,8 @@
     }
     pre_state_ = kPreNone;
     pre_used_++;
+    if (pre_lead_) lead_used_++;
+    pre_lead_ = false;
     return true;
 }
 
diff --git a/linear-programming-vanderbei_amd/csrc/kkt_knobs.h b/linear-programming-vanderbei_amd/csrc/kkt_knobs.h
--- a/linear-programming-vanderbei_amd/csrc/kkt_knobs.h
+++ b/linear-programming-vanderbei_amd/csrc/kkt_knobs.h
@@ -10,6 +10,8 @@
 constexpr int kTailVisitBlocks = 4;
 constexpr int kTailVisitLatest = 4;
 constexpr int kLongQCol = 256;
+constexpr int kTrailHelpers = 8;
+constexpr int kTrailMinBlocks = 4;
 
 struct KktKnobs {
 
@@ -18,6 +20,9 @@
     bool sf = true;
     bool overlap = true;
     bool prepass = true;
+    int lead_trail = -1;
+    int lead_trail_mode(int ntb) const { return lead_trail >= 0 ? lead_trail : ntb >= kTrailMinBlocks ? 2 : 0; }
+    int lead_helpers = kTrailHelpers;
     bool chain_lead = true;
     bool chain_pairs = false;
     bool tail_run = true;
@@ -82,6 +87,9 @@
         k.sf = flag("IPO_HIP_SF", true);
         k.overlap = flag("IPO_HIP_OVERLAP", true);
         k.prepass = flag("IPO_HIP_PREPASS", true);
+    k.lead_trail = num("IPO_HIP_LEAD_TRAIL", -1);
+    if (k.lead_trail < 0 || k.lead_trail > 2) k.lead_trail = -1;
+    k.lead_helpers = std::max(1, num("IPO_HIP_LEAD_HELPERS", kTrailHelpers));
         k.chain_lead = flag("IPO_HIP_CHAIN_LEAD", true);
         k.chain_pairs = flag("IPO_HIP_CHAIN_PAIRS", false);
         k.tail_run = flag("IPO_HIP_TAIL_RUN", true);
diff --git a/linear-programming-vanderbei_amd/csrc/kkt_schedule.cpp b/linear-programming-vanderbei_amd/csrc/kkt_schedule.cpp
--- a/linear-programming-vanderbei_amd/csrc/kkt_schedule.cpp
+++ b/linear-programming-vanderbei_amd/csrc/kkt_schedule.cpp
@@ -339,6 +339,12 @@
     return 0;
 }
 
+int sweep_lead_end(const std::vector<SweepStep>& fwd) {
+    for (size_t i = 0; i < fwd.size(); i++)
+        if (fwd[i].kind == kSwTailLead) return static_cast<int>(i) + 1;
+    return 0;
+}
+
 SweepSteps build_sweep_steps(const KktPlan& P, const KktKnobs& knobs, const KktPaths& paths, const SolveChunks& ch,
                              const SweepOrder& order, const SyncFreePlan& sf, bool blocked) {
     SweepSteps r;
@@ -377,6 +383,7 @@
     if (range) r.bwd.push_back({kSwSyncFree, 0, static_cast<int>(sf.items_b.size()), 0, 0});
     for (int l = top - 1; l >= 0; l--) level(l, r.bwd);
     r.split = sweep_split(r.fwd);
+    r.lead_end = sweep_lead_end(r.fwd);
     return r;
 }
 
diff --git a/linear-programming-vanderbei_amd/csrc/kkt_schedule.h b/linear-programming-vanderbei_amd/csrc/kkt_schedule.h
--- a/linear-programming-vanderbei_amd/csrc/kkt_schedule.h
+++ b/linear-programming-vanderbei_amd/csrc/kkt_schedule.h
@@ -50,8 +50,10 @@
 struct SweepSteps {
     std::vector<SweepStep> fwd, bwd;
     int split = 0;
+    int lead_end = 0;
 };
 int sweep_split(const std::vector<SweepStep>& fwd);
+int sweep_lead_end(const std::vector<SweepStep>& fwd);
 int sweep_launches(const std::vector<SweepStep>& steps);
 
 struct KktLaunch {
@@ -140,6 +142,10 @@
 
 
 constexpr inline int visit_hi(int t, int c, int K) { return c - 1 - K * (c - 1 - t); }
+constexpr inline int lead_col_target(int nt, int t) {
+    return (nt - t * kPanelCols + kTileRows - 1) / kTileRows - 1 > 1 ? (nt - t * kPanelCols + kTileRows - 1) / kTileRows - 1
+                                                                      : 1;
+}
 
 int tail_visit_tiles(int ntb, int t, int K);
 std::vector<unsigned> tail_visit_schedule(int ntb, int nt, int K, int cap, bool xcd, std::vector<int>& ptr);
diff --git a/linear-programming-vanderbei_amd/csrc/kkt_sweep.hip b/linear-programming-vanderbei_amd/csrc/kkt_sweep.hip
--- a/linear-programming-vanderbei_amd/csrc/kkt_sweep.hip
+++ b/linear-programming-vanderbei_amd/csrc/kkt_sweep.hip
@@ -1154,9 +1154,10 @@
 __device__ __forceinline__ __amdgpu_buffer_rsrc_t tail_rsrc(const double* S) {
     return __builtin_amdgcn_make_buffer_rsrc(const_cast<double*>(S), 0, 0x7fffffff, 0x00020000);
 }
+template <bool SC1 = false>
 __device__ __forceinline__ double buf_ld(__amdgpu_buffer_rsrc_t rs, int voff, int soff) {
     typedef int i32x2 __attribute__((ext_vector_type(2)));
-    const i32x2 v = __builtin_amdgcn_raw_buffer_load_b64(rs, voff, soff, 0);
+    const i32x2 v = __builtin_amdgcn_raw_buffer_load_b64(rs, voff, soff, SC1 ? 16 : 0);
     return __builtin_bit_cast(double, v);
 }
 constexpr int kLeadNT = 448;
@@ -1170,22 +1171,74 @@
     __builtin_amdgcn_fence(__ATOMIC_ACQUIRE, "workgroup", "local");
 }
 
-template <int R>
+#ifndef IPO_TRAIL_SLEEP
+#define IPO_TRAIL_SLEEP 16
+#endif
+__device__ __forceinline__ bool col_wait(const int* cdone, const int* bailp, int nt, int c, int seen) {
+    const int need = lead_col_target(nt, c);
+    int ok = 1;
+    seen = __builtin_amdgcn_readfirstlane(seen);
+    while (seen < need) {
+        if (__builtin_amdgcn_readfirstlane(sc1_load_int(bailp)) != 0) {
+            ok = 0;
+            break;
+        }
+        __builtin_amdgcn_s_sleep(IPO_TRAIL_SLEEP);
+        seen = __builtin_amdgcn_readfirstlane(sc1_load_int(cdone + c));
+    }
+    asm volatile("" ::: "memory");
+    return ok != 0;
+}
+template <int R>
+__device__ __forceinline__ bool gran_wait_bail(const gran_t* g, unsigned epoch, int lane, int nr, double (&v)[R],
+                                               const int* bailp) {
+    for (;;) {
+        bool ok = true;
+#pragma unroll
+        for (int r = 0; r < R; r++) {
+            if (lane < nr) {
+                const gran_t* q = g + ((size_t)r * 64 + lane) * 2;
+                const unsigned long long lo = __hip_atomic_load(const_cast<gran_t*>(q), __ATOMIC_RELAXED,
+                                                                __HIP_MEMORY_SCOPE_AGENT);
+                const unsigned long long hi = __hip_atomic_load(const_cast<gran_t*>(q + 1), __ATOMIC_RELAXED,
+                                                                __HIP_MEMORY_SCOPE_AGENT);
+                ok &= (lo >> 32) == epoch && (hi >> 32) == epoch;
+                v[r] = __longlong_as_double(static_cast<long long>(((hi & 0xffffffffull) << 32) | (lo & 0xffffffffull)));
+            } else {
+                v[r] = 0.0;
+            }
+        }
+        if (__all(ok)) return true;
+        if (__builtin_amdgcn_readfirstlane(sc1_load_int(bailp)) != 0) return false;
+        __builtin_amdgcn_s_sleep(IPO_POLL_SLEEP);
+    }
+}
+constexpr size_t kLeadTrailLds =
+    (2 * PC * (PC + 1) + kLeadBlocks * 2 * PC + 2 * 4 * 64) * sizeof(double) + 2 * PC * sizeof(int) + 64;
+
+template <int R, bool TRAIL = false>
 __global__ void __launch_bounds__(kLeadNT)
 k_tail_fwd_lead(PlanView p, TailView tv, SweepVecs V, const double* __restrict__ epsp, gran_t* __restrict__ gran,
-                gran_t* __restrict__ pgran, unsigned epoch, int* __restrict__ ticket, int tbase) {
+                gran_t* __restrict__ pgran, unsigned epoch, int* __restrict__ ticket, int tbase,
+                const int* __restrict__ cdone) {
     extern __shared__ double lds[];
     constexpr int K = kLeadBlocks;
     const int nt = tv.nt, tc = tv.tc, ntb = tv.ntb;
+    const int* bailp = p.flags + 2;
+    int* const abort_p = reinterpret_cast<int*>(lds + 2 * PC * (PC + 1) + K * 2 * PC + 2 * 4 * 64) + 2 * PC;
     const int tid = threadIdx.x, lane = tid & 63, wv = __builtin_amdgcn_readfirstlane(tid >> 6);
     const int g = wv <= 3 ? wv - 1 : wv - 2;
     const int pl = g * 64 + lane;
     __shared__ int role_sh;
-    if (tid == 0) role_sh = __hip_atomic_fetch_add(ticket, 1, __ATOMIC_RELAXED, __HIP_MEMORY_SCOPE_AGENT) - tbase;
-    __syncthreads();
-    const int role = role_sh;
+    if (tid == 0) {
+        role_sh = __hip_atomic_fetch_add(ticket, 1, __ATOMIC_RELAXED, __HIP_MEMORY_SCOPE_AGENT) - tbase;
+        if constexpr (TRAIL) *abort_p = 0;
+    }
+    __syncthreads();
+    int role = role_sh;
     if (wv == 4 || (wv == 6 && (R == 1 || role > 0))) return;
-    if (role > 0) {
+    while (role > 0) {
+        if (TRAIL && role + K >= ntb) return;
         const int i = role + K, k0 = i * PC, nc = min(PC, nt - k0), jend = i - K;
         double* zb = lds;
         const __amdgpu_buffer_rsrc_t rs = tail_rsrc(tv.S);
@@ -1197,24 +1250,41 @@
         for (int j0 = 0; j0 < jend; j0 += kHelpBatch) {
             double t[kHelpBatch][16];
             if (wv > 0) {
+                if constexpr (TRAIL) {
+                    bool go = true;
+                    for (int b = 0; b < kHelpBatch && go; b++) {
+                        const int c = min(j0 + b, jend - 1);
+                        go = col_wait(cdone, bailp, nt, c, sc1_load_int(cdone + c));
+                    }
+                    if (!go && lane == 0) *abort_p = 1;
+                }
 #pragma unroll
                 for (int b = 0; b < kHelpBatch; b++) {
                     const int s0 = (min(j0 + b, jend - 1) * PC + g16) * nt8;
 #pragma unroll
-                    for (int q = 0; q < 16; q++) t[b][q] = buf_ld(rs, voff, s0 + q * nt8);
+                    for (int q = 0; q < 16; q++) t[b][q] = buf_ld<TRAIL>(rs, voff, s0 + q * nt8);
                 }
             } else {
+                bool gone = false;
 #pragma unroll
                 for (int b = 0; b < kHelpBatch; b++) {
-                    if (j0 + b < jend) {
+                    if (j0 + b < jend && !gone) {
                         double zj[R];
-                        gran_wait<R>(gran + (size_t)(j0 + b) * R * 128, epoch, lane, PC, zj);
+                        if constexpr (TRAIL) {
+                            if (!gran_wait_bail<R>(gran + (size_t)(j0 + b) * R * 128, epoch, lane, PC, zj, bailp)) {
+                                if (lane == 0) *abort_p = 1;
+                                gone = true;
+                            }
+                        } else {
+                            gran_wait<R>(gran + (size_t)(j0 + b) * R * 128, epoch, lane, PC, zj);
+                        }
 #pragma unroll
                         for (int r = 0; r < R; r++) zb[(b * R + r) * PC + lane] = zj[r];
                     }
                 }
             }
             lds_sync();
+            if (TRAIL && *abort_p) return;
             if (wv > 0) {
 #pragma unroll
                 for (int b = 0; b < kHelpBatch; b++) {
@@ -1233,7 +1303,10 @@
 #pragma unroll
             for (int r = 0; r < R; r++) gran_put(part_slot(pgran, i, R, r, g, lane), epoch, acc[r]);
         }
-        return;
+        if constexpr (!TRAIL) return;
+        if (tid == 0) role_sh = __hip_atomic_fetch_add(ticket, 1, __ATOMIC_RELAXED, __HIP_MEMORY_SCOPE_AGENT) - tbase;
+        lds_sync();
+        role = role_sh;
     }
     double(*Ls)[PC][PC + 1] = reinterpret_cast<double(*)[PC][PC + 1]>(lds);
     double* zh = lds + 2 * PC * (PC + 1);
@@ -1248,6 +1321,7 @@
         long long sa = 0, st = 0, sb = 0;
 #endif
         lds_sync();
+        if (TRAIL && *abort_p) return;
         for (int i = 0; i < ntb; i++) {
             LEAD_T(t0);
             const int k0 = i * PC, nc = min(PC, nt - k0);
@@ -1270,6 +1344,7 @@
             zh[((i % K) * R + rs) * PC + lane] = lane < nc ? zr[0] : 0.0;
             zown[0] = znext;
             lds_sync();
+            if (TRAIL && *abort_p) return;
 #ifdef IPO_LEAD_STAMPS
             LEAD_T(t3);
             sa += t1 - t0; st += t2 - t1; sb += t3 - t2;
@@ -1293,7 +1368,7 @@
         for (int b = 0; b < K; b++) {
             const int s0 = (max(i - K + b, 0) * PC + g16) * nt8;
 #pragma unroll
-            for (int q = 0; q < 16; q++) t[b][q] = buf_ld(rs, voff, s0 + q * nt8);
+            for (int q = 0; q < 16; q++) t[b][q] = buf_ld<TRAIL>(rs, voff, s0 + q * nt8);
         }
     };
     auto l11_load = [&](int i, double(&t)[16], int& lvv) {
@@ -1303,9 +1378,10 @@
         for (int q = 0; q < 16; q++) {
             const int r = g + 4 * q;
             const bool ok = r < nc && lane < r;
-            t[q] = buf_ld(rs, ok ? voff : 0, min(k0 + r, nt - 1) * nt8);
-        }
-        lvv = p.live[tc + k0 + min(pl, nc - 1)];
+            t[q] = buf_ld<TRAIL>(rs, ok ? voff : 0, min(k0 + r, nt - 1) * nt8);
+        }
+        if constexpr (TRAIL) lvv = sc1_load_int(p.live + tc + k0 + min(pl, nc - 1));
+        else lvv = p.live[tc + k0 + min(pl, nc - 1)];
     };
     auto l11_store = [&](int i, const double(&t)[16], int lvv) {
         const int nc = min(PC, nt - i * PC);
@@ -1334,14 +1410,22 @@
     long long pw = 0, p3 = 0, p4 = 0;
     int polls = 0;
 #endif
+    if constexpr (TRAIL) {
+        const int c1 = min(1, ntb - 1);
+        const int s0 = sc1_load_int(cdone), s1 = sc1_load_int(cdone + c1);
+        if (!(col_wait(cdone, bailp, nt, 0, s0) && col_wait(cdone, bailp, nt, c1, s1)) && lane == 0) *abort_p = 1;
+    }
     l11_load(0, lA, vA);
     l11_store(0, lA, vA);
     load_tiles(min(1, ntb - 1), tB);
     l11_load(min(1, ntb - 1), lB, vB);
     part_load(min(1, ntb - 1));
     lds_sync();
+    if (TRAIL && *abort_p) return;
     auto step = [&](int i, double(&cur)[K][16], double(&nxt)[K][16], double(&lcur)[16], int& vcur,
                     double(&lnxt)[16], int& vnxt) {
+        int cseen = 0;
+        if constexpr (TRAIL) cseen = sc1_load_int(cdone + min(i + 2, ntb - 1));
         double acc[R];
 #pragma unroll
         for (int r = 0; r < R; r++) acc[r] = pre[r];
@@ -1365,6 +1449,12 @@
 #pragma unroll
                     for (int r = 0; r < R; r++) ok &= (praw[r][0] >> 32) == epoch && (praw[r][1] >> 32) == epoch;
                     if (__all(ok)) break;
+                    if constexpr (TRAIL) {
+                        if (__builtin_amdgcn_readfirstlane(sc1_load_int(bailp)) != 0) {
+                            if (lane == 0) *abort_p = 1;
+                            break;
+                        }
+                    }
 #ifdef IPO_LEAD_STAMPS
                     polls++;
 #endif
@@ -1399,6 +1489,9 @@
         }
         LEAD_T(u2);
         const int i2 = min(i + 2, ntb - 1);
+        if constexpr (TRAIL) {
+            if (!col_wait(cdone, bailp, nt, i2, cseen) && lane == 0) *abort_p = 1;
+        }
         load_tiles(i2, cur);
         l11_load(i2, lcur, vcur);
         part_load(i2);
@@ -1407,11 +1500,12 @@
         p3 += u2 - u0; p4 += u3 - u2;
 #endif
         lds_sync();
+        return !(TRAIL && *abort_p);
     };
     int i = 0;
     for (; i + 1 < ntb; i += 2) {
-        step(i, tA, tB, lA, vA, lB, vB);
-        step(i + 1, tB, tA, lB, vB, lA, vA);
+        if (!step(i, tA, tB, lA, vA, lB, vB)) return;
+        if (!step(i + 1, tB, tA, lB, vB, lA, vA)) return;
     }
     if (i < ntb) step(i, tA, tB, lA, vA, lB, vB);
 #ifdef IPO_LEAD_STAMPS
@@ -1865,7 +1959,9 @@
                {reinterpret_cast<const void*>(&k_tail_bwd_pair<1>), kPairBwdLds},
                {reinterpret_cast<const void*>(&k_tail_bwd_pair<2>), kPairBwdLds},
                {reinterpret_cast<const void*>(&k_tail_fwd_lead<1>), kChainLds},
-               {reinterpret_cast<const void*>(&k_tail_fwd_lead<2>), kChainLds}});
+               {reinterpret_cast<const void*>(&k_tail_fwd_lead<2>), kChainLds},
+               {reinterpret_cast<const void*>(&k_tail_fwd_lead<1, true>), static_cast<int>(kLeadTrailLds)},
+               {reinterpret_cast<const void*>(&k_tail_fwd_lead<2, true>), static_cast<int>(kLeadTrailLds)}});
 }
 
 void KktDevice::dump_sf_stamps() const {
@@ -2027,7 +2123,7 @@
             lead_ticket_next_ += grid;
             hipLaunchKernelGGL(k_tail_fwd_lead<R>, dim3(grid), dim3(kLeadNT), kChainLds, s, pv, tv, V, epsp,
                                dChainGran_.get(), dChainGran_.get() + static_cast<size_t>(plan_.ntb) * 2 * 128,
-                               ++chain_epoch_, dlead_ticket_.get(), tb);
+                               ++chain_epoch_, dlead_ticket_.get(), tb, static_cast<const int*>(nullptr));
 #ifdef IPO_LEAD_STAMPS
             if (chain_epoch_ % 64 == 41) {
                 double st[8][4];
@@ -2085,6 +2181,24 @@
     else run_sweep_steps<1>(h_.sweep.fwd, true, dZ_.get(), epsp, 0, split, q);
 }
 
+void KktDevice::launch_lead_trail(int R, hipStream_t s, bool beside) {
+    const PlanView pv = plan_view();
+    const TailView tv = tail_view();
+    const SweepVecs V{dZ_.get(), static_cast<size_t>(T_), dYbuf_.get(), h_.ybuf_stride};
+    const int nhb = std::max(0, plan_.ntb - 1 - kLeadBlocks);
+    const int grid = 1 + (beside ? std::min(nhb, knobs_.lead_helpers) : nhb);
+    const double* epsp = dScal_.get() + 4;
+    gran_t* gran = dChainGran_.get();
+    gran_t* pgran = gran + static_cast<size_t>(plan_.ntb) * 2 * 128;
+    int* cdone = run_cdone();
+    if (R == 2)
+        hipLaunchKernelGGL((k_tail_fwd_lead<2, true>), dim3(grid), dim3(kLeadNT), kLeadTrailLds, s, pv, tv, V, epsp, gran,
+                           pgran, ++chain_epoch_, cdone + plan_.ntb, 0, static_cast<const int*>(cdone));
+    else
+        hipLaunchKernelGGL((k_tail_fwd_lead<1, true>), dim3(grid), dim3(kLeadNT), kLeadTrailLds, s, pv, tv, V, epsp, gran,
+                           pgran, ++chain_epoch_, cdone + plan_.ntb, 0, static_cast<const int*>(cdone));
+}
+
 int KktDevice::sf_tbase(int d, int nitems, hipStream_t s) {
     const long long draw = static_cast<long long>(nitems) + std::min(sf_grid_, nitems);
     if (sf_ticket_next_[d] + draw > (1LL << 30)) {
```

Result: faster. 310.0 iterations/s (median of 6 runs) (+3.7%).
